# TiagoMSSantos/MobileRayTracer

Measured on AMD Instinct MI355X. Metric: Mrays/s + ms/frame, Conference OBJ 1920×1080 4spp, 1/2/4/8 GPU, higher is better.
Workload: dtype f32; 1 GPU; conference_1920x1080_4spp_pathtracer_depth5; rendered_pixels=2058240, spp=4, max_depth=5, samples_light=1, parallelism=single GPU

## Files before the change

### __graft_entry__.py

```python
import os
import subprocess
import sys

HERE = os.path.dirname(os.path.abspath(__file__))
if HERE not in sys.path:
    sys.path.insert(0, HERE)


def build() -> None:
    jobs = str(min(16, os.cpu_count() or 1))
    subprocess.run(["make", "-j", jobs, "-C", os.path.join(HERE, "mobileraytracer_amd", "csrc")], check=True)
    subprocess.run(["make", "-C", os.path.join(HERE, "oracle")], check=True)
    subprocess.run(["make", "-C", os.path.join(HERE, "tests", "cabi")], check=True)
    from mobileraytracer_amd import scenes
    scenes.conference()
    scenes.conference_flat()
    import mobileraytracer_amd
    from mobileraytracer_amd import _native
    _native.lib()


def smoke() -> None:
    import numpy as np
    import mobileraytracer_amd as m
    from oracle import oracle as O

    cfg = m.Config(width=64, height=64, shader=1, sceneIndex=0, device=0)
    with m.Renderer(cfg) as r:
        bm = np.zeros(64 * 64, np.int32)
        r.render_frame(bm)
        rays = r.get_total_casted_rays()
    ref, ref_rays = O.Oracle(64, 64, 1, 0).render(threads=4)
    assert np.array_equal(bm, ref), "Whitted Cornell bitmap differs from the oracle"
    assert rays == ref_rays, (rays, ref_rays)
    cfg = m.Config(width=64, height=64, shader=2, sceneIndex=0, samplesPixel=2, device=0)
    with m.Renderer(cfg) as r:
        bm = np.zeros(64 * 64, np.int32)
        r.render_frame(bm)
        prays = r.get_total_casted_rays()
        orig, dirs, keys, pixels = r.camera_rays()
        rgb = r.shade_rays(orig[:64], dirs[:64], keys[:64]).cpu().numpy()
        for q, px in enumerate(pixels[:64:2].cpu().numpy()):
            first = O.incremental_avg([float(x) for x in rgb[2 * q]], 0, 1)
            assert O.incremental_avg([float(x) for x in rgb[2 * q + 1]], first, 2) == bm[px], "shaded camera rays differ"
    ref, ref_prays = O.Oracle(64, 64, 2, 0, 2).render(threads=4)
    assert np.array_equal(bm, ref), "PathTracer Cornell bitmap differs from the oracle"
    assert prays == ref_prays, (prays, ref_prays)
    print("smoke ok: Cornell Whitted and PathTracer bit-exact, rays", rays, prays)


if __name__ == "__main__":
    build()
    smoke()
```

### include/mobilert_amd.h

```cpp
#ifndef MOBILERT_AMD_H
#define MOBILERT_AMD_H

#include <stddef.h>
#include <stdint.h>

#ifdef __cplusplus
extern "C" {
#endif

typedef struct mrt_renderer mrt_renderer;

typedef struct mrt_config {
    int32_t width;
    int32_t height;
    int32_t threads;
    int32_t shader;
    int32_t sceneIndex;
    int32_t samplesPixel;
    int32_t samplesLight;
    int32_t repeats;
    int32_t accelerator;
    int32_t printStdOut;
    const char *objFilePath;
    const char *mtlFilePath;
// ... 71 lines not shown
    int64_t worstCase;
    int64_t rayCap[MRT_QUEUE_LEVELS];
    int64_t shadowCap[MRT_QUEUE_LEVELS];
    int64_t requestedRays[MRT_QUEUE_LEVELS];
    int64_t requestedShadows[MRT_QUEUE_LEVELS];
} mrt_queue_info;

typedef struct mrt_queue_plan_request {
    int32_t levels;
    int32_t branching;
    int32_t samplesPixel;
    int32_t samplesLight;
    int32_t textured;
    int32_t segments;
    int32_t growthPct;
    int32_t slack;
    int32_t worstCase;
    int32_t hasDemand;
    int64_t pixelSlots;
    int64_t pathBudget;
    int64_t byteBudget;
    int32_t overflowMask;
    int32_t reserved;
    int64_t demandChunkSlots;
    int64_t demandPaths;
    int64_t segDemand[MRT_QUEUE_LEVELS];
    int64_t shadowSegDemand[MRT_QUEUE_LEVELS];
    int64_t prevChunkSlots;
    int64_t prevSegCap[MRT_QUEUE_LEVELS];
    int64_t prevShadowSegCap[MRT_QUEUE_LEVELS];
} mrt_queue_plan_request;

typedef struct mrt_queue_plan {
    int64_t chunkSlots;
    int64_t segCap[MRT_QUEUE_LEVELS];
    int64_t shadowSegCap[MRT_QUEUE_LEVELS];
    int64_t bytes;
    int64_t worstCase;
} mrt_queue_plan;

typedef struct mrt_blob {
    const char *name;
    const uint8_t *bytes;
    int64_t size;
} mrt_blob;

const char *mrt_last_error(void);
const char *mrt_build_stamp(void);
int mrt_create(const mrt_config *cfg, mrt_renderer **out);
int mrt_create_from_memory(const mrt_config *cfg, const char *obj, int64_t objLen, const char *mtl, int64_t mtlLen,
                           const char *cam, int64_t camLen, const mrt_blob *textures, int32_t nTextures,
                           mrt_renderer **out);
int64_t mrt_preview_arrays(const mrt_renderer *r, float *vertices, float *colors, float *camera);
void mrt_destroy(mrt_renderer *r);
int mrt_render_frame(mrt_renderer *r, int32_t *bitmap);
int mrt_render_frame_device(mrt_renderer *r, int32_t *d_bitmap, int32_t *d_packed, void *stream);
int mrt_unpack_gathered(mrt_renderer *r, const int32_t *d_gathered, int32_t *d_bitmap, void *stream);
int mrt_stop_render(mrt_renderer *r);
int32_t mrt_get_sample(const mrt_renderer *r);
uint64_t mrt_get_total_casted_rays(const mrt_renderer *r);
int mrt_get_scene_info(const mrt_renderer *r, mrt_scene_info *info);
int mrt_set_profiling(mrt_renderer *r, int32_t flags);
int mrt_get_frame_stats(const mrt_renderer *r, mrt_frame_stats *stats);
int mrt_get_queue_info(const mrt_renderer *r, mrt_queue_info *out, size_t size);
int64_t mrt_wave_log(mrt_renderer *r, uint64_t *out);
int mrt_set_camera(mrt_renderer *r, int32_t kind, const float *position, const float *lookAt, const float *up,
                   float a, float b);
int mrt_set_pixel_sampler(mrt_renderer *r, int32_t kind, float value);
int mrt_set_max_point(mrt_renderer *r, const float *maxPoint);
typedef struct mrt_view {
    int32_t kind;
    float position[3], lookAt[3], up[3];
    float a, b;
} mrt_view;
int mrt_render_views(mrt_renderer *r, const mrt_view *views, int32_t nViews, int32_t *bitmaps);
int mrt_render_views_device(mrt_renderer *r, const mrt_view *views, int32_t nViews,
                            int32_t *d_bitmaps, int32_t *d_packed, void *stream);
int mrt_set_tuning(mrt_renderer *r, int32_t key, int32_t value);
int mrt_get_tuning(const mrt_renderer *r, int32_t key, int32_t *value);
int mrt_primary_hits(mrt_renderer *r, int32_t *kind, int32_t *index, float *t);
int64_t mrt_triangle_bvh(const mrt_config *cfg, float *boxes, int32_t *offsets, int32_t *counts, int32_t *order);
int64_t mrt_walk_tree(const mrt_config *cfg, uint32_t *nodes, float *grid, int32_t *root);
int mrt_walk_stack(const mrt_config *cfg, int32_t *out);
int64_t mrt_plan_spill(int64_t threads, int32_t stackNeed, int64_t availBytes);
int64_t mrt_regular_grid(const mrt_config *cfg, int32_t kind, float *world, int32_t *start, int32_t *items);
int mrt_grid_box_test(int32_t kind, const float *prim, const float *box);
int64_t mrt_decode_texture(const char *path, int32_t *dims, uint8_t *texels);
int mrt_plan_queues(const mrt_queue_plan_request *request, mrt_queue_plan *plan);

int mrt_sample_tables(float *shader, float *sampler, float *trig);

int mrt_kat_slab(const float *boxes, const float *orig, const float *dir, int32_t n, int32_t *out);
int mrt_kat_triangle(const float *tris, const float *orig, const float *dir, int32_t n, int32_t *hit, float *t);
int mrt_kat_accumulate(const float *rgb, int32_t nSlots, int32_t spp, int32_t sampleBase, int32_t width,
                       int32_t height, int32_t mode, int32_t *bitmap, int32_t *launched);
int mrt_trace_rays(mrt_renderer *r, const float *orig, const float *dir, const float *dist, const int32_t *src,
                   int32_t n, int32_t any, int32_t *kind, int32_t *index, float *t);

typedef struct mrt_ray_batch {
    const float   *orig;
    const float   *dir;
    const float   *dist;
    const int32_t *src;
    int64_t origStride;
    int64_t dirStride;
    int64_t n;
} mrt_ray_batch;

int mrt_cast_rays_device(mrt_renderer *r, const mrt_ray_batch *rays, int32_t any,
                         int32_t *d_kind, int32_t *d_index, float *d_t, void *stream);

typedef struct mrt_hit_records {
    int32_t *kind; int32_t *index; float *t;
    float   *bary;
    float   *point;
    float   *normal;
    float   *texCoord;
    int32_t *material;
    float   *kd;
    float   *ks, *kt, *le;
    float   *ior;
} mrt_hit_records;

int mrt_cast_hits_device(mrt_renderer *r, const mrt_ray_batch *rays, const mrt_hit_records *out, size_t outSize,
                         void *stream);

int64_t mrt_scene_triangles(const mrt_config *cfg, float *geom, float *normals, float *texCoords, int32_t *material);
int64_t mrt_scene_planes(const mrt_config *cfg, float *normalPoint, int32_t *material);
int64_t mrt_scene_spheres(const mrt_config *cfg, float *centreSqRadius, int32_t *material);
int64_t mrt_scene_materials(const mrt_config *cfg, float *coeffs, int32_t *texture);
int64_t mrt_scene_lights(const mrt_config *cfg, int32_t *kind, float *geom, float *coeffs);


uint32_t mrt_path_key(uint32_t pixel, uint32_t sample);

typedef struct mrt_shade_batch {
    mrt_ray_batch rays;
    const uint32_t *key;
} mrt_shade_batch;

int mrt_shade_rays_device(mrt_renderer *r, const mrt_shade_batch *b, float *d_rgb, int64_t rgbStride,
                          uint64_t *raysOut, void *stream);

int64_t mrt_camera_rays_device(mrt_renderer *r, const mrt_view *view, int32_t sampleBase, int32_t spp,
                               float *d_orig, float *d_dir, uint32_t *d_key, int32_t *d_pixel, void *stream);

#ifdef __cplusplus
}
#endif

#endif
```

### mobileraytracer_amd/__init__.py

```python
import contextlib
import ctypes
import dataclasses
import threading
import time
from typing import List, Optional

import numpy as np

from . import _native

SHADER_WHITTED = 1
SHADER_PATH_TRACER = 2
ACC_BVH = 3
RAY_DEPTH_MAX = 6


@dataclasses.dataclass
class Config:
    width: int = 256
    height: int = 256
    threads: int = 1
    shader: int = SHADER_WHITTED
    sceneIndex: int = 0
    samplesPixel: int = 1
# ... 307 lines not shown
    def shade_rays(self, orig, dirs, keys=None, src=None):
        import torch

        device, n, orig, orig_stride, dirs, dir_stride = self._ray_tensors(orig, dirs)
        if keys is not None:
            if keys.device != device or keys.shape != (n,) or keys.dtype.is_floating_point:
                raise ValueError("keys: an integer tensor of shape (%d,) on %s" % (n, device))
            if keys.dtype == torch.uint32:
                keys = keys.contiguous().view(torch.int32)
            elif keys.dtype != torch.int32:
                keys = keys.to(torch.int64).to(torch.int32)
            keys = keys.contiguous()
        if src is not None:
            if src.device != device or src.shape != (n, 2):
                raise ValueError("src: a tensor of shape (%d, 2) on %s" % (n, device))
            src = src.to(torch.int32).contiguous()
        rgb = torch.empty((n, 3), dtype=torch.float32, device=device)
        if n == 0:
            return rgb
        with self._query_stream_of(device) as stream:
            self.shade_rays_device(orig.data_ptr(), dirs.data_ptr(), n, d_key=keys.data_ptr() if keys is not None else 0,
                                   d_src=src.data_ptr() if src is not None else 0, orig_stride=orig_stride,
                                   dir_stride=dir_stride, d_rgb=rgb.data_ptr(), stream=stream)
        return rgb

    def camera_rays(self, camera=None, sample_base: int = 0, spp: Optional[int] = None):
        import torch

        spp = int(spp) if spp else max(1, self.config.samplesPixel)
        n = self.scene_info()["pixelSlots"] * spp
        device = torch.device("cuda", self.config.device if self.config.device >= 0 and not self.config.devices
                              else torch.cuda.current_device())
        orig = torch.empty((n, 3), dtype=torch.float32, device=device)
        dirs = torch.empty((n, 3), dtype=torch.float32, device=device)
        keys = torch.empty(n, dtype=torch.int32, device=device).view(torch.uint32)
        pixels = torch.empty(n, dtype=torch.int32, device=device)
        if n == 0:
            return orig, dirs, keys, pixels
        view = self._views([camera]) if camera is not None else None
        got = self._lib.mrt_camera_rays_device(self._h, view, int(sample_base), spp, orig.data_ptr(), dirs.data_ptr(),
                                               keys.data_ptr(), pixels.data_ptr(),
                                               ctypes.c_void_p(torch.cuda.current_stream(device).cuda_stream or None))
        if got != n:
            _native.check(-1 if got < 0 else 0)
            raise RuntimeError("mrt_camera_rays_device returned %d paths, %d expected" % (got, n))
        return orig, dirs, keys, pixels

    def close(self) -> None:
        if getattr(self, "_h", None):
            self._lib.mrt_destroy(self._h)
            self._h = None

    def __del__(self):
        self.close()

    def __enter__(self):
        return self

    def __exit__(self, *exc):
        self.close()


def walk_tree(config: Config):
    lib = _native.lib()
    c = config.to_c()
    n = lib.mrt_walk_tree(ctypes.byref(c), None, None, None)
    if n < 0:
        raise RuntimeError(lib.mrt_last_error().decode())
    grid = np.empty(6, np.float32)
    root = np.empty(3, np.int32)
    lib.mrt_walk_tree(ctypes.byref(c), None, _ptr(grid), _ptr(root))
    nodes = np.empty((n, 4 * int(root[2])), np.uint32)
    if lib.mrt_walk_tree(ctypes.byref(c), _ptr(nodes), _ptr(grid), _ptr(root)) != n:
        raise RuntimeError(lib.mrt_last_error().decode())
    return nodes, grid, root


def walk_stack(config: Config) -> dict:
    out = np.zeros(6, np.int32)
    c = config.to_c()
    _native.check(_native.lib().mrt_walk_stack(ctypes.byref(c), _ptr(out)))
    return {"need": int(out[0]), "quantized": bool(out[1]), "refDepth": int(out[2]), "walkDepth": int(out[3]),
            "wideDepth": int(out[4]), "spillDepth": int(out[5])}


def plan_spill(threads: int, stack_need: int, avail_bytes: int = 0) -> int:
    n = _native.lib().mrt_plan_spill(int(threads), int(stack_need), int(avail_bytes))
    if n < 0:
        raise RuntimeError(_native.lib().mrt_last_error().decode())
    return int(n)


def triangle_bvh(config: Config):
    lib = _native.lib()
    c = config.to_c()
    n = lib.mrt_triangle_bvh(ctypes.byref(c), None, None, None, None)
    if n < 0:
        raise RuntimeError(lib.mrt_last_error().decode())
    boxes = np.empty((n, 6), np.float32)
    off, cnt = np.empty(n, np.int32), np.empty(n, np.int32)
    order = np.full((n + 1) // 2, -1, np.int32)
    n2 = lib.mrt_triangle_bvh(ctypes.byref(c), _ptr(boxes), _ptr(off), _ptr(cnt), _ptr(order))
    if n2 != n:
        raise RuntimeError(lib.mrt_last_error().decode())
    return boxes, off, cnt, order[:int(cnt[0])] if n == 1 else order


def _scene_arrays(name, config, shapes):
    lib = _native.lib()
    fn = getattr(lib, name)
    c = config.to_c()
    n = fn(ctypes.byref(c), *([None] * len(shapes)))
    if n < 0:
        raise RuntimeError(lib.mrt_last_error().decode())
    arrays = [np.zeros((n,) + shape, dtype) for dtype, shape in shapes]
    if fn(ctypes.byref(c), *[_ptr(a) for a in arrays]) != n:
        raise RuntimeError(lib.mrt_last_error().decode())
    return arrays


def scene_triangles(config: Config):
    return tuple(_scene_arrays("mrt_scene_triangles", config, [(np.float32, (3, 3)), (np.float32, (3, 3)),
                                                               (np.float32, (3, 2)), (np.int32, ())]))


def scene_planes(config: Config):
    return tuple(_scene_arrays("mrt_scene_planes", config, [(np.float32, (2, 3)), (np.int32, ())]))


def scene_spheres(config: Config):
    return tuple(_scene_arrays("mrt_scene_spheres", config, [(np.float32, (4,)), (np.int32, ())]))


def scene_materials(config: Config):
    return tuple(_scene_arrays("mrt_scene_materials", config, [(np.float32, (13,)), (np.int32, ())]))


def scene_lights(config: Config):
    return tuple(_scene_arrays("mrt_scene_lights", config, [(np.int32, ()), (np.float32, (3, 3)), (np.float32, (13,))]))


def plan_queues(levels: int, branching: int, pixel_slots: int, samples_pixel: int = 1, samples_light: int = 1,
                textured: bool = False, path_budget: int = 0, byte_budget: int = 0, growth_pct: int = 0,
                slack: int = -1, worst_case: bool = False, demand: Optional[dict] = None,
                previous: Optional[dict] = None) -> dict:
    q = _native.MrtQueuePlanRequest()
    q.levels, q.branching, q.samplesPixel, q.samplesLight = levels, branching, samples_pixel, samples_light
    q.textured, q.segments, q.growthPct, q.slack = int(textured), 0, growth_pct, slack
    q.worstCase, q.pixelSlots, q.pathBudget, q.byteBudget = int(worst_case), pixel_slots, path_budget, byte_budget
    if demand is not None:
        q.hasDemand = 1
        q.overflowMask = int(demand["mask"])
        q.demandChunkSlots = int(demand["chunkSlots"])
        q.demandPaths = int(demand["paths"])
        for i, v in enumerate(demand["seg"]):
            q.segDemand[i] = int(v)
        for i, v in enumerate(demand["shadowSeg"]):
            q.shadowSegDemand[i] = int(v)
    if previous is not None:
        q.prevChunkSlots = int(previous["chunkSlots"])
        for i, v in enumerate(previous["segCap"]):
            q.prevSegCap[i] = int(v)
        for i, v in enumerate(previous["shadowSegCap"]):
            q.prevShadowSegCap[i] = int(v)
    plan = _native.MrtQueuePlan()
    _native.check(_native.lib().mrt_plan_queues(ctypes.byref(q), ctypes.byref(plan)))
# ... 121 lines not shown
```

### mobileraytracer_amd/_native.py

```python
import ctypes
import os

_HERE = os.path.dirname(os.path.abspath(__file__))
LIB_PATH = os.environ.get("MOBILERT_LIB") or os.path.join(_HERE, "libmobilert_amd.so")

EXPORTED_SYMBOLS = (
    "mrt_last_error", "mrt_build_stamp", "mrt_create", "mrt_destroy", "mrt_render_frame", "mrt_render_frame_device",
    "mrt_unpack_gathered", "mrt_stop_render", "mrt_get_sample", "mrt_get_total_casted_rays",
    "mrt_get_scene_info", "mrt_set_profiling", "mrt_get_frame_stats", "mrt_primary_hits", "mrt_set_tuning",
    "mrt_get_tuning", "mrt_triangle_bvh", "mrt_walk_tree", "mrt_decode_texture", "mrt_kat_slab", "mrt_kat_triangle",
    "mrt_trace_rays", "mrt_sample_tables", "mrt_regular_grid", "mrt_grid_box_test", "mrt_create_from_memory",
    "mrt_preview_arrays", "mrt_wave_log", "mrt_set_camera", "mrt_set_pixel_sampler", "mrt_set_max_point",
    "mrt_android_read_file", "mrt_android_initialize", "mrt_android_render_into_bitmap",
    "mrt_android_render_into_bitmap_cb", "mrt_android_wait_render", "mrt_android_start_render",
    "mrt_android_stop_render", "mrt_android_finish_render", "mrt_android_state", "mrt_android_fps",
    "mrt_android_time_renderer", "mrt_android_sample", "mrt_android_number_of_lights", "mrt_android_resize",
    "mrt_android_vertices", "mrt_android_colors", "mrt_android_camera", "mrt_android_reset",
    "mrt_get_queue_info", "mrt_plan_queues", "mrt_render_views", "mrt_render_views_device",
    "mrt_kat_accumulate", "mrt_cast_rays_device", "mrt_walk_stack", "mrt_plan_spill",
    "mrt_path_key", "mrt_shade_rays_device", "mrt_camera_rays_device",
    "mrt_cast_hits_device", "mrt_scene_triangles", "mrt_scene_planes", "mrt_scene_spheres", "mrt_scene_materials",
    "mrt_scene_lights",
    "RayTrace", "stopRender",
)


class MrtConfig(ctypes.Structure):
    _fields_ = [
        ("width", ctypes.c_int32), ("height", ctypes.c_int32), ("threads", ctypes.c_int32),
        ("shader", ctypes.c_int32), ("sceneIndex", ctypes.c_int32), ("samplesPixel", ctypes.c_int32),
        ("samplesLight", ctypes.c_int32), ("repeats", ctypes.c_int32), ("accelerator", ctypes.c_int32),
        ("printStdOut", ctypes.c_int32),
        ("objFilePath", ctypes.c_char_p), ("mtlFilePath", ctypes.c_char_p), ("camFilePath", ctypes.c_char_p),
        ("maxDepth", ctypes.c_int32), ("rankIndex", ctypes.c_int32), ("rankCount", ctypes.c_int32),
        ("device", ctypes.c_int32), ("cull", ctypes.c_int32), ("maxPathsPerPass", ctypes.c_int32),
        ("progressive", ctypes.c_int32), ("devices", ctypes.POINTER(ctypes.c_int32)), ("deviceCount", ctypes.c_int32),
    ]


class MrtAndroidConfig(ctypes.Structure):
    _fields_ = [(n, ctypes.c_int32) for n in (
        "scene", "shader", "accelerator", "width", "height", "samplesPixel", "samplesLight")] + [
        ("objFilePath", ctypes.c_char_p)]


class MrtBlob(ctypes.Structure):
    _fields_ = [("name", ctypes.c_char_p), ("bytes", ctypes.c_char_p), ("size", ctypes.c_int64)]


class MrtView(ctypes.Structure):
    _fields_ = [("kind", ctypes.c_int32), ("position", ctypes.c_float * 3), ("lookAt", ctypes.c_float * 3),
                ("up", ctypes.c_float * 3), ("a", ctypes.c_float), ("b", ctypes.c_float)]


class MrtRayBatch(ctypes.Structure):
    _fields_ = [("orig", ctypes.c_void_p), ("dir", ctypes.c_void_p), ("dist", ctypes.c_void_p), ("src", ctypes.c_void_p),
                ("origStride", ctypes.c_int64), ("dirStride", ctypes.c_int64), ("n", ctypes.c_int64)]


HIT_FIELDS = (("kind", "int32", 1), ("index", "int32", 1), ("t", "float32", 1), ("bary", "float32", 2),
              ("point", "float32", 3), ("normal", "float32", 3), ("texCoord", "float32", 2), ("material", "int32", 1),
              ("kd", "float32", 3), ("ks", "float32", 3), ("kt", "float32", 3), ("le", "float32", 3), ("ior", "float32", 1))


class MrtHitRecords(ctypes.Structure):
    _fields_ = [(name, ctypes.c_void_p) for name, _, _ in HIT_FIELDS]


class MrtShadeBatch(ctypes.Structure):
    _fields_ = [("rays", MrtRayBatch), ("key", ctypes.c_void_p)]


class MrtSceneInfo(ctypes.Structure):
    _fields_ = [(n, ctypes.c_int64) for n in (
        "triangles", "lights", "planes", "spheres", "materials", "triangleNodes", "triangleBvhDepth",
        "pixelSlots", "pixelSlotsMax", "deviceBytes", "shadowStreamConcurrent", "shadowStreamsTried", "deviceCount")]


class MrtFrameStats(ctypes.Structure):
    _fields_ = [
        ("rays", ctypes.c_uint64), ("shadowRays", ctypes.c_uint64), ("primaryRays", ctypes.c_uint64),
        ("nodeRecords", ctypes.c_uint64), ("triTests", ctypes.c_uint64),
        ("shadowNodeRecords", ctypes.c_uint64), ("shadowTriTests", ctypes.c_uint64),
        ("traceMs", ctypes.c_double), ("shadowMs", ctypes.c_double), ("frameMs", ctypes.c_double),
        ("traceLaunches", ctypes.c_int64), ("shadowLaunches", ctypes.c_int64),
        ("shadeMs", ctypes.c_double),
        ("levelRays", ctypes.c_uint64 * 16), ("levelShadowRays", ctypes.c_uint64 * 16),
        ("levelTraceMs", ctypes.c_double * 16), ("levelShadowMs", ctypes.c_double * 16),
        ("maxNodeRecordsPerRay", ctypes.c_uint64),
        ("walkedRays", ctypes.c_uint64), ("shadedVertices", ctypes.c_uint64), ("shadeLaunches", ctypes.c_int64),
        ("leafRecords", ctypes.c_uint64), ("shadowLeafRecords", ctypes.c_uint64),
        ("levelNodeRecords", ctypes.c_uint64 * 16), ("levelTriTests", ctypes.c_uint64 * 16),
        ("levelLeafRecords", ctypes.c_uint64 * 16),
        ("fusedMs", ctypes.c_double), ("fusedLaunches", ctypes.c_int64),
        ("levelShadedVertices", ctypes.c_uint64 * 16),
        ("shadowOccluded", ctypes.c_uint64),
        ("walkPhases", ctypes.c_uint64 * 16),
        ("packetWaveRecords", ctypes.c_uint64 * 3),
    ]


QUEUE_LEVELS = 16


class MrtQueueInfo(ctypes.Structure):
    _fields_ = [(n, ctypes.c_int64) for n in (
        "chunkSlots", "passes", "queueBytes", "budgetBytes", "replans", "replansLastFrame", "worstCase")] + [
        (n, ctypes.c_int64 * QUEUE_LEVELS) for n in ("rayCap", "shadowCap", "requestedRays", "requestedShadows")]


class MrtQueuePlanRequest(ctypes.Structure):
    _fields_ = [(n, ctypes.c_int32) for n in (
        "levels", "branching", "samplesPixel", "samplesLight", "textured", "segments", "growthPct", "slack",
        "worstCase", "hasDemand")] + [
        ("pixelSlots", ctypes.c_int64), ("pathBudget", ctypes.c_int64), ("byteBudget", ctypes.c_int64),
        ("overflowMask", ctypes.c_int32), ("reserved", ctypes.c_int32),
        ("demandChunkSlots", ctypes.c_int64), ("demandPaths", ctypes.c_int64),
        ("segDemand", ctypes.c_int64 * QUEUE_LEVELS), ("shadowSegDemand", ctypes.c_int64 * QUEUE_LEVELS),
        ("prevChunkSlots", ctypes.c_int64),
        ("prevSegCap", ctypes.c_int64 * QUEUE_LEVELS), ("prevShadowSegCap", ctypes.c_int64 * QUEUE_LEVELS)]


class MrtQueuePlan(ctypes.Structure):
    _fields_ = [("chunkSlots", ctypes.c_int64), ("segCap", ctypes.c_int64 * QUEUE_LEVELS),
                ("shadowSegCap", ctypes.c_int64 * QUEUE_LEVELS), ("bytes", ctypes.c_int64),
                ("worstCase", ctypes.c_int64)]


def _preload_torch_hip_runtime():
    import importlib.util
    spec = importlib.util.find_spec("torch")
    if spec is None or not spec.origin:
        return
    rt = os.path.join(os.path.dirname(spec.origin), "lib", "libamdhip64.so")
    if os.path.exists(rt):
        ctypes.CDLL(rt, mode=ctypes.RTLD_GLOBAL)


def load_library(path=LIB_PATH):
    if not os.path.exists(path):
        raise ImportError(
            f"{path} is missing: build it with `python -c 'import __graft_entry__ as g; g.build()'` "
            "(the MI355X path has no CPU fallback)")
    _preload_torch_hip_runtime()
    lib = ctypes.CDLL(path)
    P = ctypes.POINTER
    vp = ctypes.c_void_p
    sig = {
        "mrt_last_error": (ctypes.c_char_p, []),
        "mrt_build_stamp": (ctypes.c_char_p, []),
        "mrt_create": (ctypes.c_int, [P(MrtConfig), P(vp)]),
        "mrt_destroy": (None, [vp]),
        "mrt_render_frame": (ctypes.c_int, [vp, vp]),
        "mrt_render_frame_device": (ctypes.c_int, [vp, vp, vp, vp]),
        "mrt_render_views": (ctypes.c_int, [vp, P(MrtView), ctypes.c_int32, vp]),
        "mrt_render_views_device": (ctypes.c_int, [vp, P(MrtView), ctypes.c_int32, vp, vp, vp]),
        "mrt_unpack_gathered": (ctypes.c_int, [vp, vp, vp, vp]),
        "mrt_stop_render": (ctypes.c_int, [vp]),
        "mrt_get_sample": (ctypes.c_int32, [vp]),
        "mrt_get_total_casted_rays": (ctypes.c_uint64, [vp]),
        "mrt_get_scene_info": (ctypes.c_int, [vp, P(MrtSceneInfo)]),
        "mrt_set_profiling": (ctypes.c_int, [vp, ctypes.c_int32]),
        "mrt_get_frame_stats": (ctypes.c_int, [vp, P(MrtFrameStats)]),
        "mrt_get_queue_info": (ctypes.c_int, [vp, vp, ctypes.c_size_t]),
        "mrt_plan_queues": (ctypes.c_int, [P(MrtQueuePlanRequest), P(MrtQueuePlan)]),
        "mrt_wave_log": (ctypes.c_int64, [vp, vp]),
        "mrt_primary_hits": (ctypes.c_int, [vp, vp, vp, vp]),
        "mrt_set_tuning": (ctypes.c_int, [vp, ctypes.c_int32, ctypes.c_int32]),
        "mrt_get_tuning": (ctypes.c_int, [vp, ctypes.c_int32, ctypes.POINTER(ctypes.c_int32)]),
        "mrt_triangle_bvh": (ctypes.c_int64, [vp, vp, vp, vp, vp]),
        "mrt_walk_tree": (ctypes.c_int64, [vp, vp, vp, vp]),
        "mrt_walk_stack": (ctypes.c_int, [vp, vp]),
        "mrt_plan_spill": (ctypes.c_int64, [ctypes.c_int64, ctypes.c_int32, ctypes.c_int64]),
        "mrt_decode_texture": (ctypes.c_int64, [ctypes.c_char_p, vp, vp]),
        "mrt_regular_grid": (ctypes.c_int64, [vp, ctypes.c_int32, vp, vp, vp]),
        "mrt_grid_box_test": (ctypes.c_int, [ctypes.c_int32, vp, vp]),
        "mrt_create_from_memory": (ctypes.c_int, [P(MrtConfig), ctypes.c_char_p, ctypes.c_int64, ctypes.c_char_p,
                                                  ctypes.c_int64, ctypes.c_char_p, ctypes.c_int64, vp, ctypes.c_int32,
                                                  P(vp)]),
        "mrt_preview_arrays": (ctypes.c_int64, [vp, vp, vp, vp]),
        "mrt_set_camera": (ctypes.c_int, [vp, ctypes.c_int32, vp, vp, vp, ctypes.c_float, ctypes.c_float]),
        "mrt_set_pixel_sampler": (ctypes.c_int, [vp, ctypes.c_int32, ctypes.c_float]),
        "mrt_set_max_point": (ctypes.c_int, [vp, vp]),
        "mrt_android_read_file": (None, [ctypes.c_char_p, ctypes.c_char_p, ctypes.c_int64]),
        "mrt_android_initialize": (ctypes.c_int32, [P(MrtAndroidConfig)]),
        "mrt_android_render_into_bitmap": (None, [vp, ctypes.c_int32]),
        "mrt_android_render_into_bitmap_cb": (None, [vp, ctypes.c_int32, vp, vp]),
        "mrt_android_wait_render": (None, []),
        "mrt_android_start_render": (None, [ctypes.c_int32]),
        "mrt_android_stop_render": (None, [ctypes.c_int32]),
        "mrt_android_finish_render": (None, []),
        "mrt_android_state": (ctypes.c_int32, []),
        "mrt_android_fps": (ctypes.c_float, []),
        "mrt_android_time_renderer": (ctypes.c_int64, []),
        "mrt_android_sample": (ctypes.c_int32, []),
        "mrt_android_number_of_lights": (ctypes.c_int32, []),
        "mrt_android_resize": (ctypes.c_int32, [ctypes.c_int32]),
        "mrt_android_vertices": (ctypes.c_int64, [vp]),
        "mrt_android_colors": (ctypes.c_int64, [vp]),
        "mrt_android_camera": (ctypes.c_int64, [vp]),
        "mrt_android_reset": (None, []),
        "mrt_sample_tables": (ctypes.c_int, [vp, vp, vp]),
        "mrt_kat_slab": (ctypes.c_int, [vp, vp, vp, ctypes.c_int32, vp]),
        "mrt_kat_triangle": (ctypes.c_int, [vp, vp, vp, ctypes.c_int32, vp, vp]),
        "mrt_kat_accumulate": (ctypes.c_int, [vp] + [ctypes.c_int32] * 6 + [vp, P(ctypes.c_int32)]),
        "mrt_trace_rays": (ctypes.c_int, [vp, vp, vp, vp, vp, ctypes.c_int32, ctypes.c_int32, vp, vp, vp]),
        "mrt_cast_rays_device": (ctypes.c_int, [vp, P(MrtRayBatch), ctypes.c_int32, vp, vp, vp, vp]),
        "mrt_cast_hits_device": (ctypes.c_int, [vp, P(MrtRayBatch), P(MrtHitRecords), ctypes.c_size_t, vp]),
        "mrt_scene_triangles": (ctypes.c_int64, [vp, vp, vp, vp, vp]),
        "mrt_scene_planes": (ctypes.c_int64, [vp, vp, vp]),
        "mrt_scene_spheres": (ctypes.c_int64, [vp, vp, vp]),
        "mrt_scene_materials": (ctypes.c_int64, [vp, vp, vp]),
        "mrt_scene_lights": (ctypes.c_int64, [vp, vp, vp, vp]),
        "mrt_path_key": (ctypes.c_uint32, [ctypes.c_uint32, ctypes.c_uint32]),
        "mrt_shade_rays_device": (ctypes.c_int, [vp, P(MrtShadeBatch), vp, ctypes.c_int64, P(ctypes.c_uint64), vp]),
        "mrt_camera_rays_device": (ctypes.c_int64, [vp, P(MrtView), ctypes.c_int32, ctypes.c_int32, vp, vp, vp, vp, vp]),
    }
    for name, (res, args) in sig.items():
        if os.environ.get("MOBILERT_LIB") and not hasattr(lib, name):
            continue
        fn = getattr(lib, name)
        fn.restype = res
        fn.argtypes = args
    return lib


_LIB = None


def lib():
    global _LIB
    if _LIB is None:
        _LIB = load_library()
    return _LIB


def source_stamp():
    import hashlib
    d = os.path.join(_HERE, "csrc")
    srcs = ["mrt_scene.cpp", "mrt_grid.cpp", "mrt_texture.cpp", "mrt_android.cpp", "mrt_queue_plan.cpp", "mrt_kernels.hip",
            "mrt_renderer.hip",
            "mrt_common.hpp", "mrt_device.hpp", "mrt_kernels.hpp", "mrt_trace_ww.hpp", "mrt_trace_packet.hpp",
            "mrt_scene.hpp", "mrt_queue_plan.hpp", "../../include/mobilert_amd.h", "../../include/mobilert_amd.hpp",
            "../../include/mobilert_android.h"]
    h = hashlib.sha256()
    for f in srcs:
        with open(os.path.join(d, f), "rb") as fh:
            h.update(fh.read())
    return h.hexdigest()[:16]


def build_is_current(library=None):
    return (library or lib()).mrt_build_stamp().decode() == source_stamp()


# ... 4 lines not shown
```

### mobileraytracer_amd/csrc/mrt_kernels.hip

```cpp
#include "mrt_kernels.hpp"
#include "mrt_trace_ww.hpp"
#include "mrt_trace_packet.hpp"

#include <algorithm>
#include <atomic>
#include <utility>

namespace mrt {

__device__ __forceinline__ int laneId() { return static_cast<int>(threadIdx.x & 63u); }

__device__ __forceinline__ int waveExclusiveScan(int v, int* total) {
    const int lane = laneId();
    int x = v;
#pragma unroll
    for (int off = 1; off < 64; off <<= 1) {
        const int y = __shfl_up(x, off, 64);
        if (lane >= off) x += y;
    }
    *total = __shfl(x, 63, 64);
    return x - v;
}

__device__ __forceinline__ int waveAlloc(int* counter, int n) {
// ... 51 lines not shown
__device__ __forceinline__ void cameraRayOf(const GCamera& c, float u, float v, float devU, float devV, uint32_t key,
                                            float4* o4, float4* d4) {
    v3 origin, dir;
    if (c.kind == 1) {
        const float rf = (u - 0.5F) * c.hFov;
        const v3 right = c.right * rf + c.right * devU;
        const float uf = (0.5F - v) * c.vFov;
        const v3 up = c.up * uf + c.up * devV;
        origin = (c.position + right) + up;
        dir = c.direction;
    } else {
        const float rf = fastArcTan(c.hFov * (u - 0.5F)) + devU;
        const v3 right = c.right * rf;
        const float uf = fastArcTan(c.vFov * (0.5F - v)) + devV;
        const v3 up = c.up * uf;
        const v3 dest = ((c.position + c.direction) + right) + up;
        origin = c.position;
        dir = normalize(dest - c.position);
    }
    *o4 = make_float4(origin.x, origin.y, origin.z, bitsf(key));
    *d4 = make_float4(dir.x, dir.y, dir.z, bitsf(kNoPrim));
}
static_assert(sizeof(GCamera) == 64, "cameraRay reads a view's camera as 16 dwords");
template <bool kViews = false>
__device__ __forceinline__ void cameraRay(const RaygenArgs& a, int p, float4* o4, float4* d4) {
    int slot = a.slotBase + p / a.spp;
    int view = 0;
    if constexpr (kViews) {
        view = slot / a.viewSlots;
        slot -= view * a.viewSlots;
    }
    const int s = p % a.spp;
    int x, y;
    slotToXY(a.map, slot, &x, &y);
    const uint32_t pixelIndex = static_cast<uint32_t>(y * a.width + x);
    const uint32_t key = pathKey(pixelIndex, static_cast<uint32_t>(a.sampleBase + s));
    const float invW = 1.0F / static_cast<float>(a.width);
    const float invH = 1.0F / static_cast<float>(a.height);
    const float pixW = 0.5F / static_cast<float>(a.width);
    const float pixH = 0.5F / static_cast<float>(a.height);
    const float u = static_cast<float>(x) * invW;
    const float v = static_cast<float>(y) * invH;
    float r1 = a.constJitter, r2 = a.constJitter;
    if (a.tableJitter != 0) {
        const float2 j = a.jitter[sampleBlock(key, 0u)];
        r1 = j.x;
        r2 = j.y;
    }
    const float devU = (r1 - 0.5F) * 2.0F * pixW;
    const float devV = (r2 - 0.5F) * 2.0F * pixH;
    if constexpr (kViews) {
        const int first = __builtin_amdgcn_readfirstlane(view);
        if (__ballot(view != first) == 0) {
            ConstU32* const w = (ConstU32*)(a.cams) + 16 * first;
            const float4 c0 = sload4f(w), c1 = sload4f(w + 4), c2 = sload4f(w + 8), c3 = sload4f(w + 12);
            pinSgprs(c0);
            pinSgprs(c1);
            pinSgprs(c2);
            pinSgprs(c3);
            const GCamera c{v3{c0.x, c0.y, c0.z}, v3{c0.w, c1.x, c1.y}, v3{c1.z, c1.w, c2.x}, v3{c2.y, c2.z, c2.w},
                            c3.x, c3.y, __float_as_int(c3.z), 0};
            cameraRayOf(c, u, v, devU, devV, key, o4, d4);
        } else {
            const GCamera c = a.cams[view];
            cameraRayOf(c, u, v, devU, devV, key, o4, d4);
        }
    } else {
        cameraRayOf(a.cam, u, v, devU, devV, key, o4, d4);
    }
}

template <bool kViews>
__global__ __launch_bounds__(256) void k_raygen(RaygenArgs a, Level lv, int* counters) {
    const int p = static_cast<int>(blockIdx.x * blockDim.x + threadIdx.x);
    if (p == 0) denseCounts(counters, 1, false, a.nPaths, lv.segCap);
    if (p >= a.nPaths) return;
    float4 o4, d4;
    cameraRay<kViews>(a, p, &o4, &d4);
    lv.rO[p] = o4;
    lv.rD[p] = d4;
    lv.tree[p] = 1u;
}

constexpr int kWalkThreads = 256;

template <bool kCount>
__device__ __forceinline__ void reduceCounts(const TravCount& cnt, unsigned long long* stats, int nodesStat,
                                             int trisStat, int leavesStat) {
    unsigned long long n = cnt.nodes, t = cnt.tris, l = cnt.leaves;
    for (int off = 32; off > 0; off >>= 1) {
        n += __shfl_down(n, off, 64);
        t += __shfl_down(t, off, 64);
        l += __shfl_down(l, off, 64);
    }
    if (laneId() == 0) {
        atomicAdd(stats + nodesStat, n);
        atomicAdd(stats + trisStat, t);
        atomicAdd(stats + leavesStat, l);
    }
}

__device__ __forceinline__ void reducePhases(const TravCount& cnt, unsigned long long* stats, int kind) {
    const uint32_t v[6] = {cnt.innerIters, cnt.innerLanes, cnt.leafIters, cnt.leafLanes, cnt.triIters, cnt.triLanes};
#pragma unroll
    for (int k = 0; k < 6; ++k) {
        unsigned long long x = v[k];
        for (int off = 32; off > 0; off >>= 1) x += __shfl_down(x, off, 64);
        if (laneId() == 0 && x != 0) atomicAdd(stats + kStatPhases + 6 * kind + k, x);
    }
    const uint32_t w[2] = {cnt.innerIdle, cnt.innerDone};
#pragma unroll
    for (int k = 0; k < 2; ++k) {
        unsigned long long x = w[k];
        for (int off = 32; off > 0; off >>= 1) x += __shfl_down(x, off, 64);
        if (laneId() == 0 && x != 0) atomicAdd(stats + kStatPhases + 12 + 2 * kind + k, x);
    }
}

__device__ __forceinline__ void waveLog(const TravCount& cnt, unsigned long long* stats, int kind, int level,
                                        unsigned long long t0) {
    unsigned long long n = cnt.nodes, r = cnt.rays;
    for (int off = 32; off > 0; off >>= 1) {
        n += __shfl_down(n, off, 64);
        r += __shfl_down(r, off, 64);
    }
    const int wave = static_cast<int>(blockIdx.x * (kWalkThreads / 64) + threadIdx.x / 64);
    if (laneId() == 0 && wave < kWaveLogWaves && level < kMaxLevels) {
        unsigned long long* e = stats + kNumStats + ((static_cast<size_t>(kind) * kMaxLevels + level) * kWaveLogWaves + wave) * 4;
        e[0] = t0;
        e[1] = __builtin_amdgcn_s_memrealtime();
        e[2] = r;
        e[3] = n;
    }
}

template <int kCull>
__device__ __forceinline__ auto makeWalkStack(int2* ldsStack, int2* gstack, int gdepth) {
    if constexpr (kCull == kCullFast || kCull == kCullCertified)
        return makeKeyStack<kWalkThreads>(ldsStack, gstack, gdepth);
    else
        return makeRefStack<kWalkThreads>(ldsStack, gstack, gdepth);
}

#ifndef MRT_WALK_WAVES
#define MRT_WALK_WAVES 6
#endif
#ifndef MRT_SHADOW_WAVES
#define MRT_SHADOW_WAVES MRT_WALK_WAVES
#endif
template <bool kCount, int kVariant, int kCull>
__global__ __launch_bounds__(kWalkThreads, MRT_WALK_WAVES) void k_trace(DScene s, Level lv, int* counters, int level,
                                                            int2* gstack, int gdepth, unsigned long long* stats) {
    __shared__ int2 ldsStack[kWalkStack * kWalkThreads];
    auto st = makeWalkStack<kCull>(ldsStack, gstack, gdepth);
    const unsigned long long t0 = kCount ? __builtin_amdgcn_s_memrealtime() : 0ull;
    const SegMap map = segMap(counters, level, false, lv.segCap);
    int* fetch = counters + kCntFetchShards + level * kMaxFetchShards * kFetchStride;
    TravCount cnt{0u, 0u};
    if (kVariant == 1) {
        __shared__ QNode4 ldsTop[kWalkTop];
        __shared__ int tailBest[kWalkThreads];
        stageTop<kWalkThreads>(s, ldsTop);
        traceWhileWhile<false, kCount, kCull>(s, lv.rO, lv.rD, lv.hit, map, fetch, st, &cnt, ldsTop, tailBest);
    }
    while (kVariant == 0) {
        int base = 0;
        if (laneId() == 0) base = atomicAdd(fetch, 64);
        base = __shfl(base, 0, 64);
        if (base >= map.total()) break;
        const int v = base + laneId();
        if (v < map.total()) {
            const int i = map.phys(v);
            const float4 o4 = lv.rO[i];
            const float4 d4 = lv.rD[i];
            const Best b = closestHit(s, xyz(o4), xyz(d4), fbits(d4.w), st, &cnt);
            lv.hit[i] = make_float4(b.t, b.u, b.v, bitsf(b.code));
        }
    }
    if (kCount) {
        reduceCounts<kCount>(cnt, stats, kStatNodes, kStatTris, kStatLeaves);
        reduceCounts<kCount>(cnt, stats, kStatLevelNodes + level - 1, kStatLevelTris + level - 1, kStatLevelLeaves + level - 1);
        reducePhases(cnt, stats, 0);
        atomicMax(stats + kStatMaxNodesRay, static_cast<unsigned long long>(cnt.rayMax));
        waveLog(cnt, stats, 0, level, t0);
    }
}

template <bool kViews>
struct PacketRaysStore {
    const RaygenArgs* a;
    Level lv;
    __device__ __forceinline__ void operator()(int i, float4* o4, float4* d4) const {
        cameraRay<kViews>(*a, i, o4, d4);
        if (a->storeRays != 0) {
            lv.rO[i] = *o4;
            lv.rD[i] = *d4;
            lv.tree[i] = 1u;
        }
    }
};

template <bool kCount, int kCull, int kGen>
__global__ __launch_bounds__(kWalkThreads, kGen ? 7 : 8) void k_trace_packet(DScene s, Level lv, int* counters, int level,
                                                                   int2* gstack, int gdepth, unsigned long long* stats,
                                                                   RaygenArgs ra) {
    __shared__ int2 ldsStack[kWalkStack * kWalkThreads];
    __shared__ int waveStacks[kWalkThreads / 64][kPacketStack];
    auto st = makeWalkStack<kCull>(ldsStack, gstack, gdepth);
    const unsigned long long t0 = kCount ? __builtin_amdgcn_s_memrealtime() : 0ull;
// ... 1481 lines not shown
```

### mobileraytracer_amd/csrc/mrt_kernels.hpp

```cpp
#pragma once

#include "mrt_device.hpp"

namespace mrt {

constexpr int kShaderWhitted = 1;
constexpr int kShaderPathTracer = 2;
constexpr int kShaderDepthMap = 3;
constexpr int kShaderDiffuse = 4;
constexpr int kShaderNoShadows = 5;
constexpr int kMaxLevels = 16;
constexpr int kTraceVariants = 2;
constexpr int kDefaultTraceVariant = 1;
constexpr int kAccNaive = 1;
constexpr int kAccGrid = 2;
constexpr int kAccBVH = 3;
constexpr int kTopNodesMax = 64 * 4 / kWalkWidth;

#ifndef MRT_QUEUE_SEGS
#define MRT_QUEUE_SEGS 8
#endif
constexpr int kQueueSegs = MRT_QUEUE_SEGS;
constexpr int kCntSegStride = 64;
constexpr int kCntPairs = 0;
constexpr int kCntOverflow = kQueueSegs * kCntSegStride;
constexpr int kPacketStack = 128;
#ifndef MRT_WALK_CURSORS
#define MRT_WALK_CURSORS 8
#endif
constexpr int kMaxFetchShards = MRT_WALK_CURSORS;
constexpr int kFetchStride = 32;
constexpr int kCntFetchShards = kCntOverflow + kFetchStride;
constexpr int kNumCounters = kCntFetchShards + 2 * kMaxLevels * kMaxFetchShards * kFetchStride;
MRT_HD constexpr int cntRays(int level, int seg = 0) { return kCntPairs + seg * kCntSegStride + 2 * (level - 1); }
MRT_HD constexpr int cntShadows(int level, int seg = 0) { return kCntPairs + seg * kCntSegStride + 2 * level + 1; }
static_assert(kQueueSegs >= 1 && kQueueSegs <= kMaxFetchShards, "queue segments: one work cursor each at most");
static_assert(cntShadows(kMaxLevels) < kCntSegStride, "a segment's pairs within its line");

constexpr int kStatRays = 0;
constexpr int kStatShadowRays = 1;
constexpr int kStatPrimary = 2;
constexpr int kStatNodes = 3;
constexpr int kStatTris = 4;
constexpr int kStatOverflow = 5;
constexpr int kStatNodesShadow = 6;
constexpr int kStatTrisShadow = 7;
constexpr int kStatLevelRays = 8;
constexpr int kStatLevelShadows = 8 + kMaxLevels;
constexpr int kStatMaxNodesRay = 8 + 2 * kMaxLevels;
constexpr int kStatSkipped = kStatMaxNodesRay + 1;
constexpr int kStatShaded = kStatSkipped + 1;
constexpr int kStatShadeLaunches = kStatShaded + 1;
constexpr int kStatLeaves = kStatShadeLaunches + 1;
constexpr int kStatLeavesShadow = kStatLeaves + 1;
constexpr int kStatLevelNodes = kStatLeavesShadow + 1;
constexpr int kStatLevelTris = kStatLevelNodes + kMaxLevels;
constexpr int kStatLevelLeaves = kStatLevelTris + kMaxLevels;
constexpr int kStatLevelShaded = kStatLevelLeaves + kMaxLevels;
constexpr int kStatOccluded = kStatLevelShaded + kMaxLevels;
constexpr int kStatPhases = kStatOccluded + 1;
constexpr int kStatPacket = kStatPhases + 16;
constexpr int kStatReqSegRays = kStatPacket + 3;
constexpr int kStatReqSegShadows = kStatReqSegRays + kMaxLevels;
constexpr int kStatReqRays = kStatReqSegShadows + kMaxLevels;
constexpr int kStatReqShadows = kStatReqRays + kMaxLevels;
constexpr int kNumStats = kStatReqShadows + kMaxLevels;
constexpr int kWaveLogWaves = 8192;
constexpr int kWaveLogEntries = 2 * kMaxLevels * kWaveLogWaves * 4;

struct Level {
    float4* rO;
    float4* rD;
    uint32_t* tree;
    float4* hit;
    int4* vtx;
    float4* res;
    float4* sO;
    float4* sD;
    float4* sC;
    float4* kd;
    float4* last;
    int cap;
    int shadowCap;
    int segCap;
    int shadowSegCap;
};

struct TexLevel {
    const int4* vtx;
    const float4* kd;
    const float4* last;
    int cap;
    int pad;
};

struct PixelMap {
    const int4* rect;
    const int* prefix;
    int nUnits;
    int pad;
// ... 164 lines not shown
```

### mobileraytracer_amd/csrc/mrt_renderer.hip

```cpp
#include <algorithm>
#include <atomic>
#include <chrono>
#include <cmath>
#include <condition_variable>
#include <functional>
#include <cstdio>
#include <cstdlib>
#include <cstring>
#include <deque>
#include <exception>
#include <future>
#include <memory>
#include <mutex>
#include <stdexcept>
#include <map>
#include <sstream>
#include <string>
#include <thread>
#include <unordered_map>
#include <vector>

#include "mobilert_amd.h"
#include "mobilert_amd.hpp"
#include "mrt_kernels.hpp"
#include "mrt_queue_plan.hpp"
#include "mrt_scene.hpp"

namespace {

#define MRT_HIP(x)                                                                              \
    do {                                                                                        \
        const hipError_t e_ = (x);                                                              \
        if (e_ != hipSuccess) throw std::runtime_error(std::string(#x) + ": " + hipGetErrorString(e_)); \
    } while (0)

thread_local std::string gLastError;

struct DeviceMem {
    std::vector<void*> ptrs;
    size_t total = 0;
    template <class T>
    T* alloc(size_t n) {
        if (n == 0) n = 1;
        void* p = nullptr;
        MRT_HIP(hipMalloc(&p, n * sizeof(T)));
        ptrs.push_back(p);
        total += n * sizeof(T);
        return static_cast<T*>(p);
    }
    template <class T>
    T* upload(const std::vector<T>& v, hipStream_t st) {
        T* p = alloc<T>(v.size());
        if (!v.empty()) MRT_HIP(hipMemcpyAsync(p, v.data(), v.size() * sizeof(T), hipMemcpyHostToDevice, st));
        return p;
    }
    void release() {
        for (void* p : ptrs) (void)hipFree(p);
        ptrs.clear();
        total = 0;
    }
    ~DeviceMem() { release(); }
};

#ifndef MRT_RAY_ROT_SWEEPS
#define MRT_RAY_ROT_SWEEPS 1
#endif
constexpr int kRayRotSweeps = MRT_RAY_ROT_SWEEPS;
constexpr size_t kFrameTreeCache = 4;
struct FrameTree {
    std::vector<mrt::HBVHNode> nodes;
    std::vector<double> cost;
};
struct Fnv64 {
    uint64_t h = 1469598103934665603ull;
    void add(const void* p, size_t n) {
        const auto* b = static_cast<const unsigned char*>(p);
        for (size_t i = 0; i < n; ++i) h = (h ^ b[i]) * 1099511628211ull;
    }
    template <class T>
    void pod(const T& v) { add(&v, sizeof(v)); }
};
std::vector<mrt::HBVHNode> frameWalkTree(const std::vector<mrt::HBVHNode>& wn, const mrt::HScene& sc, const mrt::GCamera& cam,
                                         int width, int height, int maxDepth, std::vector<double>* cost) {
    cost->clear();
    const char* ce = std::getenv("MOBILERT_COLLAPSE");
    if (ce != nullptr && (std::string(ce) == "area" || std::string(ce) == "greedy")) return wn;
    if (wn.empty() || sc.triangles.empty() || width <= 0 || height <= 0) {
        cost->assign(wn.size(), 0.0);
        return wn;
    }
    const char* re = std::getenv("MOBILERT_RAY_ROT");
    const int sweeps = re != nullptr ? std::atoi(re) : kRayRotSweeps;
    Fnv64 f;
    f.add(wn.data(), wn.size() * sizeof(mrt::HBVHNode));
    for (const mrt::HTriangle& t : sc.triangles) {
        f.pod(t.AC);
        f.pod(t.AB);
        f.pod(t.A);
        f.pod(t.mat);
    }
    for (const mrt::HMaterial& m : sc.materials) {
        f.pod(m.Le);
        f.pod(m.Kd);
        f.pod(m.Ks);
    }
    for (const mrt::HLight& l : sc.lights) {
        f.pod(l.kind);
        f.pod(l.tri.A);
        f.pod(l.tri.AB);
        f.pod(l.tri.AC);
    }
    f.pod(cam);
    const int dims[4] = {width, height, maxDepth, sweeps};
    f.pod(dims);
    using Entry = std::shared_ptr<const FrameTree>;
    static std::mutex mu;
    static std::unordered_map<uint64_t, std::shared_future<Entry>> cache;
    static std::deque<uint64_t> order;
    std::promise<Entry> mine;
    std::shared_future<Entry> pending;
    {
        std::lock_guard<std::mutex> lock(mu);
        const auto it = cache.find(f.h);
        if (it != cache.end()) {
            pending = it->second;
        } else {
            cache.emplace(f.h, mine.get_future().share());
            order.push_back(f.h);
            while (order.size() > kFrameTreeCache) {
                cache.erase(order.front());
                order.pop_front();
            }
        }
    }
    if (pending.valid()) {
        const Entry e = pending.get();
        *cost = e->cost;
        return e->nodes;
    }
    try {
        auto e = std::make_shared<FrameTree>();
        const std::vector<mrt::SampleRay> rays = mrt::sampleFrameRays(wn, sc, cam, maxDepth);
        e->nodes = sweeps > 0 ? mrt::rotateForRays(wn, rays, sweeps) : wn;
        e->cost = mrt::sampleRayNodeCosts(e->nodes, rays);
        mine.set_value(e);
        *cost = e->cost;
        return e->nodes;
    } catch (...) {
        mine.set_exception(std::current_exception());
        std::lock_guard<std::mutex> lock(mu);
        cache.erase(f.h);
        order.erase(std::remove(order.begin(), order.end(), f.h), order.end());
        throw;
    }
}

int bvhDepth(const std::vector<mrt::HBVHNode>& nodes) {
    if (nodes.empty()) return 0;
    int best = 0;
    std::vector<std::pair<int, int>> st{{0, 1}};
    while (!st.empty()) {
        const auto [i, d] = st.back();
        st.pop_back();
        best = std::max(best, d);
        const mrt::HBVHNode& n = nodes[static_cast<size_t>(i)];
        if (n.numPrimitives == 0 && nodes.size() > 1) {
            st.push_back({n.indexOffset, d + 1});
            st.push_back({n.indexOffset + 1, d + 1});
        }
    }
    return best;
}

int wideDepth(bool quantized, const mrt::GRoot& root, const std::vector<mrt::QNode4>& qn) {
    int depth4 = 0;
    std::vector<std::pair<int32_t, int>> w;
    if (quantized && root.count > 0 && root.ref >= 0) w.push_back({root.ref, 1});
    while (!w.empty()) {
        const auto [i, dep] = w.back();
        w.pop_back();
        depth4 = std::max(depth4, dep);
        for (int32_t c : qn[static_cast<size_t>(i)].ref)
            if (c >= 0 && c != mrt::kEmptyChild) w.push_back({c, dep + 1});
    }
    return depth4;
}

int walkStackNeed(int binaryDepth, int depth4) {
    return std::max(binaryDepth + 2, (mrt::kWalkWidth - 1) * depth4 + 2);
}

int spillDepth(int stackNeed) { return std::max(1, stackNeed - mrt::kLdsStackMin); }

float4 f4(mrt::v3 v, float w) { return make_float4(v.x, v.y, v.z, w); }
float asFloat(int32_t i) {
    float f;
    std::memcpy(&f, &i, 4);
    return f;
}

}

std::vector<int32_t> mrt::parseDeviceList(const char* s) {
    std::vector<int32_t> out;
    if (s == nullptr) return out;
    std::string item;
    std::istringstream in(s);
    while (std::getline(in, item, ',')) {
        char* end = nullptr;
        const long v = std::strtol(item.c_str(), &end, 10);
        if (item.empty() || end != item.c_str() + item.size() || v < 0 || v > 0x7fffffffL)
            throw std::runtime_error(std::string("MOBILERT_DEVICES: bad ordinal '") + item + "'");
        out.push_back(static_cast<int32_t>(v));
    }
    return out;
}

namespace {

class ShardPool {
public:
    explicit ShardPool(const std::vector<int>& devices) : n_(static_cast<int>(devices.size())), err_(devices.size()) {
        for (int i = 1; i < n_; ++i) th_.emplace_back([this, i, d = devices[static_cast<size_t>(i)]] { loop(i, d); });
    }
    ~ShardPool() {
        {
            std::lock_guard<std::mutex> lock(mu_);
            quit_ = true;
        }
        wake_.notify_all();
        for (std::thread& t : th_) t.join();
    }
    ShardPool(const ShardPool&) = delete;
    ShardPool& operator=(const ShardPool&) = delete;

    void run(const std::function<void(int)>& job) {
        std::lock_guard<std::mutex> serial(runMu_);
// ... 36 lines not shown
                if (bound != hipSuccess)
                    throw std::runtime_error(std::string("shard worker: hipSetDevice: ") + hipGetErrorString(bound));
                (*job)(i);
            } catch (...) {
                err_[static_cast<size_t>(i)] = std::current_exception();
            }
            {
                std::lock_guard<std::mutex> lock(mu_);
                if (--pending_ == 0) done_.notify_one();
            }
        }
    }

    const int n_;
    std::mutex runMu_, mu_;
    std::condition_variable wake_, done_;
    std::vector<std::thread> th_;
    std::vector<std::exception_ptr> err_;
    const std::function<void(int)>* job_ = nullptr;
    uint64_t gen_ = 0;
    int pending_ = 0;
    bool quit_ = false;
};

}

struct mrt_renderer {
    mrt_config cfg{};
    std::string objPath, mtlPath, camPath;
    int maxDepth = mrt::kRayDepthMaxDefault;
    int shader = mrt::kShaderWhitted;
    int nLevels = 1;
    mrt::v3 maxPoint{1.0F, 1.0F, 1.0F};
    int pixelSampler = -1;
    float pixelConst = 0.5F;
    int rankIndex = 0, rankCount = 1;
    int device = 0;
    int shadowConcurrent = 0;
    int shadowTries = 0;
    std::vector<hipStream_t> spareStreams;
    unsigned long long* spinTimes = nullptr;
    hipEvent_t joinIn = nullptr, joinOut = nullptr;

    mrt::GCamera cam{};
    mrt::DScene ds{};
    std::vector<int32_t> triOrder, planeOrder, sphereOrder;
    int64_t nTri = 0, nLights = 0, nPlanes = 0, nSpheres = 0, nMats = 0, nTriNodes = 0;
    int triDepth = 0, maxBvhDepth = 0;
    int stackNeed = 0;

    std::vector<std::vector<int4>> unitsByRank;
    std::vector<std::vector<int>> prefixByRank;
    std::vector<mrt::PixelMap> mapByRank;
    int nSlots = 0, maxSlots = 0;

    DeviceMem sceneMem, queueMem, frameMem;
    struct Pipe {
        mrt::Level levels[mrt::kMaxLevels]{};
        mrt::TexLevel* texLevels = nullptr;
        int* counters = nullptr;
        unsigned long long* stats = nullptr;
        int2* gstack = nullptr;
        int2* gstackShadow = nullptr;
        hipStream_t shadowStream = nullptr;
        std::vector<hipEvent_t> syncPool;
        std::vector<hipEvent_t> evPool;
        size_t evCount = 0;
    } pipe;
    int chunkSlots = 0;
    mrt_queue_plan plan{};
    int64_t planBudget = 0;
    int queueBudgetMiB = 0;
    int queueGrowthPct = mrt::kPlanGrowthPct;
    int queueSlack = mrt::kPlanSlack;
    int deviceShare = 1;
    bool planStale = false;
    int64_t replans = 0, replansFrame = 0;
    int64_t reqSegRays[mrt::kMaxLevels] = {}, reqSegShadows[mrt::kMaxLevels] = {};
    int64_t reqRays[mrt::kMaxLevels] = {}, reqShadows[mrt::kMaxLevels] = {};
    int overflowMask = 0;
    int64_t reqPaths = 0;
    int gdepth = 0;
    int traceThreads = 0, workGrid = 0;
    int cus = 0;
    int shadeGridPerCU = -1;
    int32_t* dBitmap = nullptr;
    int32_t* dBackup = nullptr;
    size_t backupN = 0;
    int views = 1;
    const mrt::GCamera* batchCams = nullptr;
    mrt::GCamera* dViewCams = nullptr;
    size_t viewCamsN = 0;
    std::vector<mrt::GCamera> hostViewCams;
    int32_t* dViewBitmaps = nullptr;
    size_t viewBitmapsN = 0;
    DeviceMem queryMem;
    mrt::QueryTables queryTables{};
    bool queryReady = false;
    int64_t planSlots = 0;
    int planSpp = 0;
    struct ShadeBatch {
        mrt::QueryRays rays;
        const uint32_t* keys;
        float* rgb;
        long long rgbStride;
        int64_t n;
    };
    const ShadeBatch* shade = nullptr;
    hipStream_t stream = nullptr;
    int overlap = 1;
    int skipLast = 1;
    int shadowGridPct = 0;
    int fuseL1Mode = -1;
    int genL1 = 2;
    int resolveAcc = 1;
    int shadeWaitsShadow = 0;
    int refill = 0;
    int64_t shadeLaunches = 0;
    bool walkSkipped = false;
    bool fusedL1 = false;
    int lastShadowRender = 1;
    int walkGridCap = 0;
    unsigned long long* hostStats = nullptr;
    bool countersClean = false, statsClean = false;

    bool keepHost = false;
    std::vector<mrt::HTriangle> hostTris;
    std::vector<mrt::HMaterial> hostMats;

    std::atomic<bool> stopFlag{false};
    std::atomic<int32_t> sample{0};
    std::atomic<uint64_t> totalRays{0};
    int profileFlags = 0;
    mrt_frame_stats last{};

    std::vector<std::unique_ptr<mrt_renderer>> peers;
    int32_t* dOwnPacked = nullptr;
    int32_t* dGathered = nullptr;
    std::unique_ptr<ShardPool> shardPool;

    ~mrt_renderer() {
        if (hostStats != nullptr) (void)hipHostFree(hostStats);
        for (hipEvent_t e : pipe.evPool) (void)hipEventDestroy(e);
        for (hipEvent_t e : pipe.syncPool) (void)hipEventDestroy(e);
        if (pipe.shadowStream != nullptr) (void)hipStreamDestroy(pipe.shadowStream);
        for (hipStream_t s : spareStreams) (void)hipStreamDestroy(s);
        if (joinIn != nullptr) (void)hipEventDestroy(joinIn);
        if (joinOut != nullptr) (void)hipEventDestroy(joinOut);
        if (stream != nullptr) (void)hipStreamDestroy(stream);
    }
};

namespace {

void frameUnits(int W, int H, int rankCount, std::vector<std::vector<int4>>* units,
                std::vector<std::vector<int>>* prefix) {
    const int tilesPerSide = static_cast<int>(std::sqrt(static_cast<double>(mrt::kNumberOfTiles)));
    const int bx = W / tilesPerSide, by = H / tilesPerSide;
    if (bx <= 0 || by <= 0) throw std::runtime_error("width and height must be >= 16 (Renderer.cpp:33-38)");
    const int domainSize = (W / bx) * (H / by);
    const int resolution = W * H;
    std::vector<int> blocks;
    for (int j = 0; j < mrt::kNumberOfTiles; ++j) {
        const float tile = static_cast<float>(j) / static_cast<float>(mrt::kNumberOfTiles);
        const int rb = static_cast<int>(::roundf(tile * static_cast<float>(domainSize)));
        if (std::find(blocks.begin(), blocks.end(), rb) == blocks.end()) blocks.push_back(rb);
    }
    std::vector<int4> all;
    std::vector<int> owner;
    for (size_t t = 0; t < blocks.size(); ++t) {
        const int rb = blocks[t];
        const int pixel = rb * bx % resolution;
        const int startY = ((pixel / W) * by) % H;
        const int startX = pixel % W;
        for (int b = 0; b * 8 < by; ++b) {
            int h = std::min(8, by - 8 * b);
            const int y0 = startY + 8 * b;
            while (h > 0 && (y0 + h - 1) * W + startX + bx - 1 >= resolution) --h;
            if (h > 0) {
                all.push_back(make_int4(startX, y0, bx, h));
                owner.push_back(static_cast<int>((t + static_cast<size_t>(b)) % static_cast<size_t>(rankCount)));
            }
        }
    }
    units->assign(static_cast<size_t>(rankCount), {});
    prefix->assign(static_cast<size_t>(rankCount), {});
    for (size_t u = 0; u < all.size(); ++u) (*units)[static_cast<size_t>(owner[u])].push_back(all[u]);
    for (int k = 0; k < rankCount; ++k) {
        int acc = 0;
        for (const int4& u : (*units)[static_cast<size_t>(k)]) {
            (*prefix)[static_cast<size_t>(k)].push_back(acc);
            acc += u.z * u.w;
        }
    }
}

int unitSlots(const std::vector<int4>& units) {
    int acc = 0;
    for (const int4& u : units) acc += u.z * u.w;
    return acc;
}

void buildUnits(mrt_renderer* r) {
    frameUnits(r->cfg.width, r->cfg.height, r->rankCount, &r->unitsByRank, &r->prefixByRank);
    r->maxSlots = 0;
    for (int k = 0; k < r->rankCount; ++k) {
        const int acc = unitSlots(r->unitsByRank[static_cast<size_t>(k)]);
        if (k == r->rankIndex) r->nSlots = acc;
        r->maxSlots = std::max(r->maxSlots, acc);
    }
    r->mapByRank.clear();
    for (int k = 0; k < r->rankCount; ++k) {
        mrt::PixelMap m{};
        m.rect = r->sceneMem.upload(r->unitsByRank[static_cast<size_t>(k)], r->stream);
        m.prefix = r->sceneMem.upload(r->prefixByRank[static_cast<size_t>(k)], r->stream);
        m.nUnits = static_cast<int>(r->unitsByRank[static_cast<size_t>(k)].size());
        r->mapByRank.push_back(m);
    }
}

void slotToXYHost(const std::vector<int4>& units, const std::vector<int>& prefix, int slot, int* x, int* y) {
    const auto it = std::upper_bound(prefix.begin(), prefix.end(), slot);
    const size_t u = static_cast<size_t>(it - prefix.begin()) - 1;
    const int off = slot - prefix[u];
    *x = units[u].x + off / units[u].w;
    *y = units[u].y + off % units[u].w;
}

void uploadScene(mrt_renderer* r, mrt::HScene& sc) {
    using namespace mrt;
    hipStream_t st = r->stream;
    std::vector<HBVHNode> pn = buildBVH(&sc.planes, &r->planeOrder);
    std::vector<HBVHNode> sn = buildBVH(&sc.spheres, &r->sphereOrder);
    std::vector<HBVHNode> tn = buildBVH(&sc.triangles, &r->triOrder);
    std::vector<double> rayCost;
    const std::vector<HBVHNode> wn =
        frameWalkTree(walkTreeOver(tn), sc, r->cam, r->cfg.width, r->cfg.height, r->maxDepth, &rayCost);
    r->nTri = static_cast<int64_t>(sc.triangles.size());
    r->nPlanes = static_cast<int64_t>(sc.planes.size());
    r->nSpheres = static_cast<int64_t>(sc.spheres.size());
    r->nLights = static_cast<int64_t>(sc.lights.size());
    r->nMats = static_cast<int64_t>(sc.materials.size());
    r->nTriNodes = static_cast<int64_t>(tn.size());
    r->triDepth = std::max(bvhDepth(tn), bvhDepth(wn));
    r->maxBvhDepth = std::max({r->triDepth, bvhDepth(pn), bvhDepth(sn)});

    if (r->keepHost) {
        r->hostTris = sc.triangles;
        r->hostMats = sc.materials;
    }
    std::vector<GNode> g;
    DScene& d = r->ds;
    const std::vector<uint32_t> conesRef = triangleConeWords(tn, sc.triangles);
    std::vector<QNode4> qn;
    d.qEnabled = toQuantizedBVH4(wn, sc.triangles.size(), &d.triRoot, kTopNodesMax, &d.triTop, &d.qgrid, &qn, nullptr,
                                 rayCost.empty() ? nullptr : &rayCost) ? 1 : 0;
    if (d.qEnabled == 0 || qn.empty()) qn.resize(1);
    d.triQNodes = r->sceneMem.upload(qn, st);
    {
        static_assert(kWalkWidth == 4, "packet nodes: 4 children");
        std::vector<float> qf(32 * qn.size(), 0.0F);
        for (size_t k = 0; k < qn.size(); ++k) {
            const QNode4& q = qn[k];
            for (int c = 0; c < kWalkWidth; ++c) {
                const uint32_t w0 = q.q[3 * c], w1 = q.q[3 * c + 1], w2 = q.q[3 * c + 2];
                const uint32_t v[6] = {w0 & 0xFFFFu, w1 & 0xFFFFu, w2 & 0xFFFFu, w0 >> 16, w1 >> 16, w2 >> 16};
                for (int j = 0; j < 6; ++j) qf[32 * k + 6 * static_cast<size_t>(c) + static_cast<size_t>(j)] = static_cast<float>(v[j]);
                std::memcpy(&qf[32 * k + 24 + static_cast<size_t>(c)], &q.ref[c], sizeof(int32_t));
            }
        }
        d.triQNodesF = r->sceneMem.upload(qf, st);
    }
    r->stackNeed = walkStackNeed(r->maxBvhDepth, wideDepth(d.qEnabled != 0, d.triRoot, qn));
    {
        std::string err;
        if (planSpillBytes(r->traceThreads, spillDepth(r->stackNeed), 0, &err) < 0) throw std::runtime_error(err);
    }
    toDeviceBVH(tn, sc.triangles.size(), &g, &d.triRootRef, 0, nullptr, &conesRef);
    {
        std::vector<float4> lb(std::max<size_t>(1, 3 * sc.triangles.size()), make_float4(0.0F, 0.0F, 0.0F, 0.0F));
        for (const HBVHNode& n : tn) {
            if (n.numPrimitives <= 0) continue;
            const size_t f = static_cast<size_t>(n.indexOffset);
            float c[6];
            leafCullRecord(sc.triangles, f, f + static_cast<size_t>(n.numPrimitives), n.box, c);
            lb[3 * f] = make_float4(n.box.mn.x, n.box.mn.y, n.box.mn.z, n.box.mx.x);
            lb[3 * f + 1] = make_float4(n.box.mx.y, n.box.mx.z, c[0], c[1]);
            lb[3 * f + 2] = make_float4(c[2], c[3], c[4], c[5]);
        }
        d.leafBoxes = r->sceneMem.upload(lb, st);
    }
    d.triNodes = r->sceneMem.upload(g, st);
    toDeviceBVH(pn, sc.planes.size(), &g, &d.planeRoot);
    d.planeNodes = r->sceneMem.upload(g, st);
    toDeviceBVH(sn, sc.spheres.size(), &g, &d.sphereRoot);
    d.sphereNodes = r->sceneMem.upload(g, st);

    std::vector<float4> v;
    v.reserve(sc.triangles.size() * 3);
    for (const HTriangle& t : sc.triangles) {
        v.push_back(f4(t.A, 0.0F));
        v.push_back(f4(t.AB, 0.0F));
        v.push_back(f4(t.AC, 0.0F));
    }
    d.triGeom = r->sceneMem.upload(v, st);
    v.clear();
    for (const HTriangle& t : sc.triangles) {
        v.push_back(f4(t.nA, asFloat(t.mat)));
        v.push_back(f4(t.nB, 0.0F));
        v.push_back(f4(t.nC, 0.0F));
    }
    d.triShade = r->sceneMem.upload(v, st);
    v.clear();
    for (const HTriangle& t : sc.triangles) {
        const bool flat = std::memcmp(&t.nA, &t.nB, sizeof(t.nA)) == 0 && std::memcmp(&t.nA, &t.nC, sizeof(t.nA)) == 0;
        v.push_back(f4(t.nA, asFloat(static_cast<int32_t>((static_cast<uint32_t>(t.mat + 1) << 1) | (flat ? 1u : 0u)))));
    }
    d.triHead = r->sceneMem.upload(v, st);
    v.clear();
    d.textured = 0;
    for (const HMaterial& m : sc.materials) d.textured += (m.texId >= 0 && !sc.textures.empty()) ? 1 : 0;
    if (d.textured != 0) {
        for (const HTriangle& t : sc.triangles) {
            v.push_back(make_float4(t.tA.x, t.tA.y, t.tB.x, t.tB.y));
            v.push_back(make_float4(t.tC.x, t.tC.y, 0.0F, 0.0F));
        }
        d.triTex = r->sceneMem.upload(v, st);
        v.clear();
        std::vector<int4> info;
        std::vector<uint8_t> bytes;
        for (const HTexture& t : sc.textures) {
            info.push_back(make_int4(t.width, t.height, t.channels, static_cast<int>(bytes.size())));
            bytes.insert(bytes.end(), t.texels.begin(), t.texels.end());
        }
        d.texInfo = r->sceneMem.upload(info, st);
        d.texels = r->sceneMem.upload(bytes, st);
    } else {
        d.triTex = nullptr;
        d.texInfo = nullptr;
        d.texels = nullptr;
// ... 1443 lines not shown
        r->ds.cull = value;
        return 0;
    }
    if (key == 3 && (value == 0 || value == 1)) {
        r->overlap = value;
        return 0;
    }
    if (key == 7 && (value == 0 || value == 1)) {
        r->skipLast = value;
        return 0;
    }
    if (key == 5 && (value == 0 || value == 1)) {
        r->ds.anyOrder = value;
        return 0;
    }
    if (key == 11 && value >= -1 && value <= 64) {
        r->shadeGridPerCU = value;
        return 0;
    }
    if (key == 10 && (value == 0 || value == 1)) {
        r->ds.leanShade = value;
        return 0;
    }
    if (key == 9 && value >= 0 && value <= 64) {
        r->refill = value;
        return 0;
    }
    if (key == 8 && (value == 0 || value == 1)) {
        r->ds.tailDonate = value;
        return 0;
    }
    if (key == 16 && (value == 0 || value == 1)) {
        if (value == 1 && r->stackNeed > mrt::kPacketStack) {
            gLastError = "packet walk: the walk tree needs a deeper stack";
            return -1;
        }
        r->ds.packet = value;
        return 0;
    }
    if (key == 17 && value >= -1 && value <= 1) {
        r->fuseL1Mode = value;
        return 0;
    }
    if (key == 27 && (value == 0 || value == 1)) {
        r->lastShadowRender = value;
        return 0;
    }
    if (key == 33 && value >= 0 && value <= 2) {
        r->genL1 = value;
        return 0;
    }
    if (key == 34 && (value == 0 || value == 1)) {
        r->resolveAcc = value;
        return 0;
    }
    if (key == 35 && (value == 0 || value == 1)) {
        r->shadeWaitsShadow = value;
        return 0;
    }

    if (key == 28 && value >= 0 && value <= 65536) {
        r->walkGridCap = value;
        return 0;
    }
    if (key == 6 && value >= 0 && value <= 100) {
        r->shadowGridPct = value;
        return 0;
    }
    if (key == 37 && value >= 0 && value <= (1 << 20)) {
        r->queueBudgetMiB = value;
        r->planStale = true;
        return 0;
    }
    if (key == 38 && value >= 1 && value <= 100000) {
        r->queueGrowthPct = value;
        r->planStale = true;
        return 0;
    }
    if (key == 39 && value >= 0 && value <= (1 << 24)) {
        r->queueSlack = value;
        r->planStale = true;
        return 0;
    }
    gLastError = "unknown tuning key/value";
    return -1;
}

int64_t mrt_triangle_bvh(const mrt_config* cfg, float* boxes, int32_t* offsets, int32_t* counts, int32_t* order) {
    using namespace mrt;
    int64_t n = -1;
    const int rc = guarded([&] {
        HScene sc;
        if (cfg->sceneIndex >= 0 && cfg->sceneIndex <= 3) {
            sc = builtinScene(cfg->sceneIndex);
        } else {
            std::string err;
            if (!loadObjScene(cfg->objFilePath ? cfg->objFilePath : "", cfg->mtlFilePath ? cfg->mtlFilePath : "", &sc,
                              &err))
                throw std::runtime_error(err);
        }
        std::vector<int32_t> perm;
        const std::vector<HBVHNode> nodes = buildBVH(&sc.triangles, &perm);
        n = static_cast<int64_t>(nodes.size());
        if (boxes == nullptr) return;
        for (size_t i = 0; i < nodes.size(); ++i) {
            const HBVHNode& b = nodes[i];
            const float v[6] = {b.box.mn.x, b.box.mn.y, b.box.mn.z, b.box.mx.x, b.box.mx.y, b.box.mx.z};
            std::memcpy(boxes + 6 * i, v, sizeof(v));
            offsets[i] = b.indexOffset;
            counts[i] = b.numPrimitives;
        }
        std::memcpy(order, perm.data(), perm.size() * sizeof(int32_t));
    });
    return rc == 0 ? n : -1;
}

int64_t mrt_scene_triangles(const mrt_config* cfg, float* geom, float* normals, float* texCoords, int32_t* material) {
    int64_t n = -1;
    const int rc = guarded([&] {
        const mrt::HScene sc = sceneOf(cfg);
        for (size_t i = 0; i < sc.triangles.size(); ++i) {
            const mrt::HTriangle& t = sc.triangles[i];
            if (geom != nullptr) {
                put3(geom + 9 * i, t.A);
                put3(geom + 9 * i + 3, t.AB);
                put3(geom + 9 * i + 6, t.AC);
            }
            if (normals != nullptr) {
                put3(normals + 9 * i, t.nA);
                put3(normals + 9 * i + 3, t.nB);
                put3(normals + 9 * i + 6, t.nC);
            }
            if (texCoords != nullptr) {
                const float tc[6] = {t.tA.x, t.tA.y, t.tB.x, t.tB.y, t.tC.x, t.tC.y};
                std::memcpy(texCoords + 6 * i, tc, sizeof(tc));
            }
            if (material != nullptr) material[i] = t.mat;
        }
        n = static_cast<int64_t>(sc.triangles.size());
    });
    return rc == 0 ? n : -1;
}

int64_t mrt_scene_planes(const mrt_config* cfg, float* normalPoint, int32_t* material) {
    int64_t n = -1;
    const int rc = guarded([&] {
        const mrt::HScene sc = sceneOf(cfg);
        for (size_t i = 0; i < sc.planes.size(); ++i) {
            if (normalPoint != nullptr) {
                put3(normalPoint + 6 * i, sc.planes[i].normal);
                put3(normalPoint + 6 * i + 3, sc.planes[i].point);
            }
            if (material != nullptr) material[i] = sc.planes[i].mat;
        }
        n = static_cast<int64_t>(sc.planes.size());
    });
    return rc == 0 ? n : -1;
}

int64_t mrt_scene_spheres(const mrt_config* cfg, float* centreSqRadius, int32_t* material) {
    int64_t n = -1;
    const int rc = guarded([&] {
        const mrt::HScene sc = sceneOf(cfg);
        for (size_t i = 0; i < sc.spheres.size(); ++i) {
            if (centreSqRadius != nullptr) {
                put3(centreSqRadius + 4 * i, sc.spheres[i].center);
                centreSqRadius[4 * i + 3] = sc.spheres[i].sqRadius;
            }
            if (material != nullptr) material[i] = sc.spheres[i].mat;
        }
        n = static_cast<int64_t>(sc.spheres.size());
    });
    return rc == 0 ? n : -1;
}

int64_t mrt_scene_materials(const mrt_config* cfg, float* coeffs, int32_t* texture) {
    int64_t n = -1;
    const int rc = guarded([&] {
        const mrt::HScene sc = sceneOf(cfg);
        for (size_t i = 0; i < sc.materials.size(); ++i) {
            if (coeffs != nullptr) putMaterial(coeffs + 13 * i, sc.materials[i]);
            if (texture != nullptr) texture[i] = sc.materials[i].texId;
        }
        n = static_cast<int64_t>(sc.materials.size());
    });
    return rc == 0 ? n : -1;
}

int64_t mrt_scene_lights(const mrt_config* cfg, int32_t* kind, float* geom, float* coeffs) {
    int64_t n = -1;
    const int rc = guarded([&] {
        const mrt::HScene sc = sceneOf(cfg);
        for (size_t i = 0; i < sc.lights.size(); ++i) {
            const mrt::HLight& l = sc.lights[i];
            const bool area = l.kind == mrt::kAreaLight;
            if (kind != nullptr) kind[i] = l.kind;
            if (geom != nullptr) {
                put3(geom + 9 * i, area ? l.tri.A : l.position);
                put3(geom + 9 * i + 3, area ? l.tri.AB : mrt::v3{0, 0, 0});
                put3(geom + 9 * i + 6, area ? l.tri.AC : mrt::v3{0, 0, 0});
            }
            if (coeffs != nullptr) putMaterial(coeffs + 13 * i, l.radiance);
        }
        n = static_cast<int64_t>(sc.lights.size());
    });
    return rc == 0 ? n : -1;
}

int64_t mrt_walk_tree(const mrt_config* cfg, uint32_t* nodes, float* grid, int32_t* root) {
    using namespace mrt;
    int64_t n = -1;
    const int rc = guarded([&] {
        HScene sc;
        const float ratio = cfg->height > 0 ? static_cast<float>(cfg->width) / static_cast<float>(cfg->height) : 1.0F;
        GCamera cam{};
        bool haveCam = true;
        if (cfg->sceneIndex >= 0 && cfg->sceneIndex <= 3) {
            sc = builtinScene(cfg->sceneIndex);
            cam = builtinCamera(cfg->sceneIndex, ratio);
        } else {
            std::string err;
            if (!loadObjScene(cfg->objFilePath ? cfg->objFilePath : "", cfg->mtlFilePath ? cfg->mtlFilePath : "", &sc,
                              &err))
                throw std::runtime_error(err);
            haveCam = loadCameraFile(cfg->camFilePath ? cfg->camFilePath : "", ratio, &cam, &err);
        }
        std::vector<int32_t> perm;
        const std::vector<HBVHNode> tn = buildBVH(&sc.triangles, &perm);
        GRoot r{};
        QGrid g{};
        std::vector<QNode4> qn;
        int top = 0;
        const int maxDepth = cfg->maxDepth > 0 ? cfg->maxDepth : kRayDepthMaxDefault;
        std::vector<double> cost;
        const std::vector<HBVHNode> wn = haveCam ? frameWalkTree(walkTreeOver(tn), sc, cam, cfg->width, cfg->height, maxDepth, &cost)
                                                 : walkTreeOver(tn);
        if (!toQuantizedBVH4(wn, sc.triangles.size(), &r, kTopNodesMax, &top, &g, &qn, nullptr,
                             cost.empty() ? nullptr : &cost))
            throw std::runtime_error("walk tree not quantizable (non-finite boxes)");
        n = static_cast<int64_t>(qn.size());
        if (nodes != nullptr) std::memcpy(nodes, qn.data(), qn.size() * sizeof(QNode4));
        if (grid != nullptr) {
            std::memcpy(grid, g.origin, sizeof(g.origin));
            std::memcpy(grid + 3, g.step, sizeof(g.step));
        }
        if (root != nullptr) {
            root[0] = r.ref;
            root[1] = r.count;
            root[2] = kWalkWidth;
        }
    });
    return rc == 0 ? n : -1;
}

int mrt_walk_stack(const mrt_config* cfg, int32_t* out) {
    using namespace mrt;
    return guarded([&] {
        HScene sc;
        const float ratio = cfg->height > 0 ? static_cast<float>(cfg->width) / static_cast<float>(cfg->height) : 1.0F;
        GCamera cam{};
        if (cfg->sceneIndex >= 0 && cfg->sceneIndex <= 3) {
            sc = builtinScene(cfg->sceneIndex);
            cam = builtinCamera(cfg->sceneIndex, ratio);
        } else {
            std::string err;
            if (!loadObjScene(cfg->objFilePath ? cfg->objFilePath : "", cfg->mtlFilePath ? cfg->mtlFilePath : "", &sc,
                              &err))
                throw std::runtime_error(err);
            if (!loadCameraFile(cfg->camFilePath ? cfg->camFilePath : "", ratio, &cam, &err)) throw std::runtime_error(err);
        }
        std::vector<int32_t> perm;
        const int otherDepth = std::max(bvhDepth(buildBVH(&sc.planes, &perm)), bvhDepth(buildBVH(&sc.spheres, &perm)));
        const std::vector<HBVHNode> tn = buildBVH(&sc.triangles, &perm);
        const int maxDepth = cfg->maxDepth > 0 ? cfg->maxDepth : kRayDepthMaxDefault;
        std::vector<double> cost;
        const std::vector<HBVHNode> wn = frameWalkTree(walkTreeOver(tn), sc, cam, cfg->width, cfg->height, maxDepth, &cost);
        GRoot root{};
        QGrid g{};
        std::vector<QNode4> qn;
        int top = 0;
        const bool quantized = toQuantizedBVH4(wn, sc.triangles.size(), &root, kTopNodesMax, &top, &g, &qn, nullptr,
                                               cost.empty() ? nullptr : &cost);
        const int depth4 = wideDepth(quantized, root, qn);
        out[0] = walkStackNeed(std::max({bvhDepth(tn), bvhDepth(wn), otherDepth}), depth4);
        out[1] = quantized ? 1 : 0;
        out[2] = bvhDepth(tn);
        out[3] = bvhDepth(wn);
        out[4] = depth4;
        out[5] = spillDepth(out[0]);
    });
}

int64_t mrt_plan_spill(int64_t threads, int32_t stackNeed, int64_t availBytes) {
    std::string err;
    const int64_t bytes = mrt::planSpillBytes(threads, spillDepth(stackNeed), availBytes, &err);
    if (bytes < 0) gLastError = err;
    return bytes;
}

int mrt_grid_box_test(int32_t kind, const float* prim, const float* box) {
    using namespace mrt;
    const HAABB b{v3{box[0], box[1], box[2]}, v3{box[3], box[4], box[5]}};
    const v3 p0{prim[0], prim[1], prim[2]}, p1{prim[3], prim[4], prim[5]};
    if (kind == 0) return boxIntersect(makeTriangle(p0, p1, v3{prim[6], prim[7], prim[8]}), b) ? 1 : 0;
    if (kind == 1) return boxIntersect(makePlane(p0, p1, -1), b) ? 1 : 0;
    if (kind == 2) return boxIntersect(makeSphere(p0, prim[3], -1), b) ? 1 : 0;
    gLastError = "grid box test: kind must be 0 (triangle), 1 (plane) or 2 (sphere)";
    return -1;
}

int64_t mrt_regular_grid(const mrt_config* cfg, int32_t kind, float* world, int32_t* start, int32_t* items) {
    using namespace mrt;
    int64_t n = -1;
    const int rc = guarded([&] {
        if (kind < 0 || kind > 2) throw std::runtime_error("regular grid: kind must be 0 (planes), 1 (spheres), 2 (triangles)");
        HScene sc;
        if (cfg->sceneIndex >= 0 && cfg->sceneIndex <= 3) {
            sc = builtinScene(cfg->sceneIndex);
        } else {
            std::string err;
            if (!loadObjScene(cfg->objFilePath ? cfg->objFilePath : "", cfg->mtlFilePath ? cfg->mtlFilePath : "", &sc,
                              &err))
                throw std::runtime_error(err);
        }
        std::vector<int32_t> order;
        HGrid g;
        if (kind == 0) {
            buildBVH(&sc.planes, &order);
            g = buildGrid(sc.planes, order);
        } else if (kind == 1) {
            buildBVH(&sc.spheres, &order);
            g = buildGrid(sc.spheres, order);
        } else {
            buildBVH(&sc.triangles, &order);
            g = buildGrid(sc.triangles, order);
        }
        n = static_cast<int64_t>(g.items.size());
        if (world != nullptr) {
            const float w[12] = {g.world.mn.x, g.world.mn.y, g.world.mn.z, g.world.mx.x, g.world.mx.y, g.world.mx.z,
                                 g.cellSize.x, g.cellSize.y, g.cellSize.z, g.cellSizeInv.x, g.cellSizeInv.y, g.cellSizeInv.z};
            std::memcpy(world, w, sizeof(w));
        }
        if (start != nullptr) std::memcpy(start, g.start.data(), g.start.size() * sizeof(int32_t));
        if (items != nullptr)
            for (size_t k = 0; k < g.items.size(); ++k) items[k] = order[static_cast<size_t>(g.items[k])];
    });
    return rc == 0 ? n : -1;
}

int64_t mrt_decode_texture(const char* path, int32_t* dims, uint8_t* texels) {
    int64_t n = -1;
    const int rc = guarded([&] {
        mrt::HTexture t;
        std::string err;
        if (!mrt::loadTextureFile(path != nullptr ? path : "", &t, &err)) throw std::runtime_error(err);
        n = static_cast<int64_t>(t.texels.size());
        if (dims != nullptr) {
            dims[0] = t.width;
            dims[1] = t.height;
            dims[2] = t.channels;
        }
        if (texels != nullptr) std::memcpy(texels, t.texels.data(), t.texels.size());
    });
    return rc == 0 ? n : -1;
}

int mrt_sample_tables(float* shader, float* sampler, float* trig) {
    return guarded([&] {
        std::vector<float> a, b, t;
        mrt::fillHaltonTable(&a, mrt::kSeedShaderTable);
        mrt::fillHaltonTable(&b, mrt::kSeedSamplerTable);
        mrt::fillHemisphereTrig(a, &t);
        if (shader != nullptr) std::memcpy(shader, a.data(), a.size() * sizeof(float));
        if (sampler != nullptr) std::memcpy(sampler, b.data(), b.size() * sizeof(float));
        if (trig != nullptr) std::memcpy(trig, t.data(), t.size() * sizeof(float));
    });
}

int mrt_get_tuning(const mrt_renderer* r, int32_t key, int32_t* value) {
    switch (key) {
        case 1: *value = r->ds.variant; return 0;
        case 2: *value = r->ds.cull; return 0;
        case 3: *value = r->overlap; return 0;
        case 7: *value = r->skipLast; return 0;
        case 5: *value = r->ds.anyOrder; return 0;
        case 6: *value = r->shadowGridPct; return 0;
        case 8: *value = r->ds.tailDonate; return 0;
        case 9: *value = r->refill; return 0;
        case 10: *value = r->ds.leanShade; return 0;
        case 11: *value = r->shadeGridPerCU; return 0;
        case 16: *value = r->ds.packet; return 0;
        case 17: *value = r->fuseL1Mode; return 0;
        case 27: *value = r->lastShadowRender; return 0;
        case 33: *value = r->genL1; return 0;
        case 34: *value = r->resolveAcc; return 0;
        case 35: *value = r->shadeWaitsShadow; return 0;
        case 28: *value = r->walkGridCap; return 0;
        case 37: *value = r->queueBudgetMiB; return 0;
        case 38: *value = r->queueGrowthPct; return 0;
        case 39: *value = r->queueSlack; return 0;
        case 40: *value = r->stackNeed; return 0;
        default: break;
    }
    gLastError = "unknown tuning key";
    return -1;
}

int mrt_get_frame_stats(const mrt_renderer* r, mrt_frame_stats* s) {
    *s = r->last;
    return 0;
}

int mrt_get_queue_info(const mrt_renderer* r, mrt_queue_info* out, size_t size) {
    using namespace mrt;
    if (r == nullptr || out == nullptr) {
        gLastError = "mrt_get_queue_info: null argument";
        return -1;
    }
    mrt_queue_info q{};
    q.chunkSlots = r->plan.chunkSlots;
    q.passes = (std::max<int64_t>(1, r->planSlots) + q.chunkSlots - 1) / std::max<int64_t>(1, q.chunkSlots);
    q.queueBytes = r->plan.bytes;
    q.budgetBytes = r->planBudget;
    q.replans = r->replans;
    q.replansLastFrame = r->replansFrame;
    q.worstCase = r->plan.worstCase;
    for (int l = 0; l < kMaxLevels && l < MRT_QUEUE_LEVELS; ++l) {
        q.rayCap[l] = l < r->nLevels ? r->plan.segCap[l] * kQueueSegs : 0;
        q.shadowCap[l] = l < r->nLevels ? r->plan.shadowSegCap[l] * kQueueSegs : 0;
        q.requestedRays[l] = r->reqRays[l];
        q.requestedShadows[l] = r->reqShadows[l];
    }
    for (const auto& p : r->peers) {
        q.queueBytes += p->plan.bytes;
        q.replans += p->replans;
        q.replansLastFrame += p->replansFrame;
        q.worstCase = std::max<int64_t>(q.worstCase, p->plan.worstCase);
    }
    std::memcpy(out, &q, std::min(size, sizeof(q)));
    return 0;
}

int mrt_plan_queues(const mrt_queue_plan_request* request, mrt_queue_plan* plan) {
    if (request == nullptr || plan == nullptr) {
        gLastError = "mrt_plan_queues: null argument";
        return -1;
    }
    std::string err;
    if (!mrt::planQueues(*request, plan, &err)) {
        gLastError = err;
        return -1;
    }
    return 0;
}

static void primaryHitsOne(mrt_renderer* r, int32_t* kind, int32_t* index, float* t);

int mrt_primary_hits(mrt_renderer* r, int32_t* kind, int32_t* index, float* t) {
    return guarded([&] {
        const size_t npx = static_cast<size_t>(r->cfg.width) * static_cast<size_t>(r->cfg.height);
        for (size_t i = 0; i < npx; ++i) {
            kind[i] = -1;
            index[i] = -1;
            t[i] = 0.0F;
        }
        for (int i = 0; i < groupSize(r); ++i) {
            mrt_renderer* p = shardOf(r, i);
            MRT_HIP(hipSetDevice(p->device));
            primaryHitsOne(p, kind, index, t);
        }
        MRT_HIP(hipSetDevice(r->device));
    });
}

static void primaryHitsOne(mrt_renderer* r, int32_t* kind, int32_t* index, float* t) {
    {
        using namespace mrt;
        hipStream_t st = r->stream;
        const auto& units = r->unitsByRank[static_cast<size_t>(r->rankIndex)];
        const auto& prefix = r->prefixByRank[static_cast<size_t>(r->rankIndex)];
        mrt_renderer::Pipe& pp = r->pipe;
        const int cap = pp.levels[1].cap;
        int32_t* dk = static_cast<int32_t*>(nullptr);
        int32_t* di = nullptr;
// ... 311 lines not shown
```

### mobileraytracer_amd/csrc/mrt_scene.cpp

```cpp
#include "mrt_scene.hpp"

#include <algorithm>
#include <limits>
#include <array>
#include <atomic>
#include <cmath>
#include <cstdlib>
#include <cstring>
#include <deque>
#include <functional>
#include <future>
#include <fstream>
#include <memory>
#include <mutex>
#include <queue>
#include <random>
#include <sstream>
#include <string>
#include <thread>
#include <unordered_map>

namespace mrt {

namespace {
// ... 969 lines not shown
        return dx * dy + dy * dz + dz * dx;
    };
    constexpr int W1 = kWalkWidth + 1;
    std::vector<double>& forest = *forestOut;
    std::vector<int8_t>& split = *splitOut;
    {
        forest.assign(nodes.size() * W1, 0.0);
        split.assign(nodes.size() * W1, 0);
        std::vector<std::pair<int32_t, bool>> post{{0, false}};
        while (!post.empty()) {
            const auto [i, done] = post.back();
            post.pop_back();
            if (!inner(i)) continue;
            const size_t ui = static_cast<size_t>(i);
            const int32_t l = nodes[ui].indexOffset, r = l + 1;
            if (!done) {
                post.push_back({i, true});
                post.push_back({l, false});
                post.push_back({r, false});
                continue;
            }
            const size_t ul = static_cast<size_t>(l) * W1, ur = static_cast<size_t>(r) * W1;
            auto best = [&](int j, int* k) {
                double c = std::numeric_limits<double>::infinity();
                for (int a = 1; a < j; ++a) {
                    const double v = forest[ul + static_cast<size_t>(a)] + forest[ur + static_cast<size_t>(j - a)];
                    if (v < c) {
                        c = v;
                        *k = a;
                    }
                }
                return c;
            };
            int kw = 1;
            const double asWide = area(i) + best(kWalkWidth, &kw);
            split[ui * W1] = static_cast<int8_t>(kw);
            forest[ui * W1 + 1] = asWide;
            for (int j = 2; j < W1; ++j) {
                int k = 1;
                const double c = best(j, &k);
                const bool self = asWide <= c;
                forest[ui * W1 + static_cast<size_t>(j)] = self ? asWide : c;
                split[ui * W1 + static_cast<size_t>(j)] = static_cast<int8_t>(self ? 0 : k);
            }
        }
    }
}

static double collapsedArea(const std::vector<HBVHNode>& nodes, int* depth) {
    *depth = 0;
    if (nodes.size() < 3 || nodes[0].numPrimitives > 0) return 0.0;
    std::vector<double> forest;
    std::vector<int8_t> split;
    collapseForests(nodes, &forest, &split);
    constexpr int W1 = kWalkWidth + 1;
    auto inner = [&](int32_t i) { return nodes[static_cast<size_t>(i)].numPrimitives == 0; };
    std::function<void(int32_t, int, std::vector<int32_t>&)> trees = [&](int32_t i, int j, std::vector<int32_t>& out) {
        const int k = inner(i) && j > 1 ? split[static_cast<size_t>(i) * W1 + static_cast<size_t>(j)] : 0;
        if (k == 0) {
            out.push_back(i);
            return;
        }
        trees(nodes[static_cast<size_t>(i)].indexOffset, k, out);
        trees(nodes[static_cast<size_t>(i)].indexOffset + 1, j - k, out);
    };
    std::vector<std::pair<int32_t, int>> st{{0, 1}};
    while (!st.empty()) {
        const auto [i, d] = st.back();
        st.pop_back();
        *depth = std::max(*depth, d);
        const int32_t l = nodes[static_cast<size_t>(i)].indexOffset;
        const int kw = split[static_cast<size_t>(i) * W1];
        std::vector<int32_t> c;
        trees(l, kw, c);
        trees(l + 1, kWalkWidth - kw, c);
        for (const int32_t k : c)
            if (inner(k)) st.push_back({k, d + 1});
    }
    return forest[1];
}

bool toQuantizedBVH4(const std::vector<HBVHNode>& nodes, size_t numPrims, GRoot* root, int topCount, int* topPlaced,
                     QGrid* grid, std::vector<QNode4>* out, std::vector<int32_t>* bvh2Of,
                     const std::vector<double>* nodeCost) {
    out->clear();
    if (bvh2Of != nullptr) bvh2Of->clear();
    if (topPlaced != nullptr) *topPlaced = 0;
    const HBVHNode& r = nodes[0];
    const float rmn[3] = {r.box.mn.x, r.box.mn.y, r.box.mn.z}, rmx[3] = {r.box.mx.x, r.box.mx.y, r.box.mx.z};
    for (int a = 0; a < 3; ++a) {
        root->bmin[a] = rmn[a];
        root->bmax[a] = rmx[a];
    }
    root->count = static_cast<int32_t>(numPrims);
    root->ref = 0;
    Quantizer qz;
    const bool gridOK = qz.init(rmn, rmx, grid);
    if (numPrims == 0) return gridOK;
    if (r.numPrimitives > 0) {
        root->ref = leafRef(r.indexOffset, r.numPrimitives);
        return gridOK;
    }
    if (!gridOK) return false;
    auto inner = [&](int32_t i) { return nodes[static_cast<size_t>(i)].numPrimitives == 0; };
    auto area = [&](int32_t i) {
        const HAABB& b = nodes[static_cast<size_t>(i)].box;
        const double dx = static_cast<double>(b.mx.x) - b.mn.x, dy = static_cast<double>(b.mx.y) - b.mn.y,
                     dz = static_cast<double>(b.mx.z) - b.mn.z;
        return dx * dy + dy * dz + dz * dx;
    };
    const char* collapseEnv = std::getenv("MOBILERT_COLLAPSE");
    const bool optimal = collapseEnv == nullptr || std::string(collapseEnv) != "greedy";
    constexpr int W1 = kWalkWidth + 1;
    std::vector<double> forest;
    std::vector<int8_t> split;
    if (optimal) collapseForests(nodes, &forest, &split, nodeCost);
    std::function<void(int32_t, int, std::vector<int32_t>&)> trees = [&](int32_t i, int j, std::vector<int32_t>& out) {
        const int k = inner(i) && j > 1 ? split[static_cast<size_t>(i) * W1 + static_cast<size_t>(j)] : 0;
        if (k == 0) {
            out.push_back(i);
            return;
        }
        trees(nodes[static_cast<size_t>(i)].indexOffset, k, out);
        trees(nodes[static_cast<size_t>(i)].indexOffset + 1, j - k, out);
    };
    std::vector<std::array<int32_t, kWalkWidth>> kids;
    std::vector<int32_t> node4Of(nodes.size(), -1);
    std::vector<int32_t> kidsBvh2{0};
    std::vector<int32_t> work{0};
    node4Of[0] = 0;
    kids.emplace_back();
    kids.back().fill(-1);
    while (!work.empty()) {
        const int32_t i = work.back();
        work.pop_back();
        const int32_t l = nodes[static_cast<size_t>(i)].indexOffset;
        std::vector<int32_t> c{l, l + 1};
        if (optimal) {
            const int kw = split[static_cast<size_t>(i) * W1];
            c.clear();
            trees(l, kw, c);
            trees(l + 1, kWalkWidth - kw, c);
        }
        while (!optimal && c.size() < static_cast<size_t>(kWalkWidth)) {
            int best = -1;
            double ba = -1.0;
            for (size_t k = 0; k < c.size(); ++k)
                if (inner(c[k]) && area(c[k]) > ba) {
                    ba = area(c[k]);
                    best = static_cast<int>(k);
                }
            if (best < 0) break;
            const int32_t cl = nodes[static_cast<size_t>(c[static_cast<size_t>(best)])].indexOffset;
            c[static_cast<size_t>(best)] = cl;
            c.insert(c.begin() + best + 1, cl + 1);
        }
        std::array<int32_t, kWalkWidth> k4;
        k4.fill(-1);
        for (size_t k = 0; k < c.size(); ++k) {
            k4[k] = c[k];
            if (inner(c[k])) {
                node4Of[static_cast<size_t>(c[k])] = static_cast<int32_t>(kids.size());
                kidsBvh2.push_back(c[k]);
                kids.emplace_back();
                kids.back().fill(-1);
                work.push_back(c[k]);
            }
        }
        kids[static_cast<size_t>(node4Of[static_cast<size_t>(i)])] = k4;
    }
    const size_t n4 = kids.size();
    std::vector<int32_t> newIdx(n4, -1), order;
    std::deque<int32_t> bfs{0};
    while (!bfs.empty() && static_cast<int>(order.size()) < topCount) {
        const int32_t j = bfs.front();
        bfs.pop_front();
        newIdx[static_cast<size_t>(j)] = static_cast<int32_t>(order.size());
        order.push_back(j);
        for (int32_t c : kids[static_cast<size_t>(j)])
            if (c >= 0 && inner(c)) bfs.push_back(node4Of[static_cast<size_t>(c)]);
    }
    if (topPlaced != nullptr) *topPlaced = static_cast<int>(order.size());
    std::vector<int32_t> dfs{0};
    while (!dfs.empty()) {
        const int32_t j = dfs.back();
        dfs.pop_back();
        if (newIdx[static_cast<size_t>(j)] < 0) {
            newIdx[static_cast<size_t>(j)] = static_cast<int32_t>(order.size());
            order.push_back(j);
        }
        const auto& k4 = kids[static_cast<size_t>(j)];
        for (int k = kWalkWidth - 1; k >= 0; --k)
            if (k4[static_cast<size_t>(k)] >= 0 && inner(k4[static_cast<size_t>(k)]))
                dfs.push_back(node4Of[static_cast<size_t>(k4[static_cast<size_t>(k)])]);
    }
    out->resize(n4);
    if (bvh2Of != nullptr) {
        bvh2Of->resize(n4);
        for (size_t k = 0; k < n4; ++k) (*bvh2Of)[k] = kidsBvh2[static_cast<size_t>(order[k])];
    }
    for (size_t k = 0; k < n4; ++k) {
        const auto& k4 = kids[static_cast<size_t>(order[k])];
        QNode4& q = (*out)[k];
        for (int c = 0; c < kWalkWidth; ++c) {
            const int32_t b = k4[static_cast<size_t>(c)];
            if (b < 0) {
                q.q[3 * c] = q.q[3 * c + 1] = q.q[3 * c + 2] = 0xFFFFu;
                q.ref[c] = kEmptyChild;
                continue;
            }
            const HBVHNode& bn = nodes[static_cast<size_t>(b)];
            const float mn[3] = {bn.box.mn.x, bn.box.mn.y, bn.box.mn.z}, mx[3] = {bn.box.mx.x, bn.box.mx.y, bn.box.mx.z};
            if (!qz.box(mn, mx, q.q + 3 * c)) {
                out->clear();
                return false;
            }
            q.ref[c] = bn.numPrimitives > 0 ? leafRef(bn.indexOffset, bn.numPrimitives)
                                             : newIdx[static_cast<size_t>(node4Of[static_cast<size_t>(b)])];
        }
    }
    root->ref = 0;
    return true;
}

namespace {
uint32_t coneWord(const std::vector<HTriangle>& tris, size_t lo, size_t hi) {
    double kMax = 1.0;
    double m[3][3] = {};
    std::vector<std::array<double, 3>> ns;
    ns.reserve(hi - lo);
    for (size_t i = lo; i < hi; ++i) {
        const HTriangle& t = tris[i];
        const double ab[3] = {t.AB.x, t.AB.y, t.AB.z}, ac[3] = {t.AC.x, t.AC.y, t.AC.z};
        const double n[3] = {ab[1] * ac[2] - ab[2] * ac[1], ab[2] * ac[0] - ab[0] * ac[2], ab[0] * ac[1] - ab[1] * ac[0]};
        const double len = std::sqrt(n[0] * n[0] + n[1] * n[1] + n[2] * n[2]);
        const double l1 = (std::fabs(ab[0]) + std::fabs(ab[1]) + std::fabs(ab[2])) *
                          (std::fabs(ac[0]) + std::fabs(ac[1]) + std::fabs(ac[2]));
        if (!(len > 0.0) || !std::isfinite(l1)) return kConeNever;
        kMax = std::max(kMax, l1 / len);
        const std::array<double, 3> u{n[0] / len, n[1] / len, n[2] / len};
        for (int r = 0; r < 3; ++r)
            for (int c = 0; c < 3; ++c) m[r][c] += u[static_cast<size_t>(r)] * u[static_cast<size_t>(c)];
        ns.push_back(u);
    }
    const double kCode = std::ceil(8.0 * std::log2(kMax) + 1e-9);
    if (ns.empty() || kCode > 126.0) return kConeNever;
    int col = 0;
    for (int c = 1; c < 3; ++c)
        if (m[c][c] > m[col][col]) col = c;
    double a[3] = {m[0][col], m[1][col], m[2][col]};
    for (int it = 0; it < 64; ++it) {
        double b[3];
        for (int r = 0; r < 3; ++r) b[r] = m[r][0] * a[0] + m[r][1] * a[1] + m[r][2] * a[2];
        const double l = std::sqrt(b[0] * b[0] + b[1] * b[1] + b[2] * b[2]);
        if (!(l > 0.0)) return kConeNever;
        for (int r = 0; r < 3; ++r) a[r] = b[r] / l;
    }
    const double s1 = std::fabs(a[0]) + std::fabs(a[1]) + std::fabs(a[2]);
    double ox = a[0] / s1, oy = a[1] / s1;
    if (a[2] < 0.0) {
        const double tx = ox;
        ox = (1.0 - std::fabs(oy)) * (tx >= 0.0 ? 1.0 : -1.0);
        oy = (1.0 - std::fabs(tx)) * (oy >= 0.0 ? 1.0 : -1.0);
    }
    const uint32_t qx = static_cast<uint32_t>(std::lround((ox + 1.0) * 0.5 * 511.0));
    const uint32_t qy = static_cast<uint32_t>(std::lround((oy + 1.0) * 0.5 * 511.0));
    const v3 dec = coneAxis(qx | (qy << 9));
    const double dl = std::sqrt(double(dec.x) * dec.x + double(dec.y) * dec.y + double(dec.z) * dec.z);
    const double ax[3] = {dec.x / dl, dec.y / dl, dec.z / dl};
    double cosMin = 1.0;
    for (const auto& u : ns) cosMin = std::min(cosMin, std::fabs(u[0] * ax[0] + u[1] * ax[1] + u[2] * ax[2]));
    const double psi = std::acos(std::min(1.0, cosMin)) + 2e-3;
    const double qCode = psi >= 1.5707963267948966 ? 127.0 : std::ceil(std::sin(psi) * 126.0 + 1e-9);
    if (qCode > 126.0) return kConeNever;
    return qx | (qy << 9) | (static_cast<uint32_t>(qCode) << 18) | (static_cast<uint32_t>(kCode) << 25);
}
}
// ... 477 lines not shown
    };
    auto closest = [&](v3 o, v3 d, float* tBest) {
        const v3 inv{1.0F / d.x, 1.0F / d.y, 1.0F / d.z};
        int best = -1;
        float bt = std::numeric_limits<float>::infinity();
        std::vector<int32_t> st{0};
        while (!st.empty()) {
            const size_t i = static_cast<size_t>(st.back());
            st.pop_back();
            if (!(entry(nodes[i].box, o, inv) < bt)) continue;
            if (inner(i)) {
                st.push_back(nodes[i].indexOffset + 1);
                st.push_back(nodes[i].indexOffset);
                continue;
            }
            for (int32_t k = 0; k < nodes[i].numPrimitives; ++k) {
                float t;
                const int32_t j = nodes[i].indexOffset + k;
                if (triHit(sc.triangles[static_cast<size_t>(j)], o, d, &t) && t < bt) {
                    bt = t;
                    best = j;
                }
            }
        }
        for (const HLight& l : sc.lights) {
            float t;
            if (l.kind == kAreaLight && triHit(l.tri, o, d, &t) && t < bt) {
                bt = t;
                best = -2;
            }
        }
        *tBest = bt;
        return best;
    };
    std::vector<const HLight*> areaLights;
    for (const HLight& l : sc.lights)
        if (l.kind == kAreaLight) areaLights.push_back(&l);
    std::mt19937 rng(0x4D525406u);
    std::uniform_real_distribution<float> U(0.0F, 1.0F);
    constexpr float camW = 0.6F, shadowW = 1.0F;
    constexpr int gx = 192, gy = 108;
    struct Path {
        v3 o, d;
        int depth;
    };
    for (int py = 0; py < gy; ++py)
        for (int px = 0; px < gx; ++px) {
            const float u = (static_cast<float>(px) + U(rng)) / static_cast<float>(gx);
            const float v = (static_cast<float>(py) + U(rng)) / static_cast<float>(gy);
            v3 o, d;
            if (cam.kind == 1) {
                o = (cam.position + cam.right * ((u - 0.5F) * cam.hFov)) + cam.up * ((0.5F - v) * cam.vFov);
                d = cam.direction;
            } else {
                const v3 dest = ((cam.position + cam.direction) + cam.right * fastArcTan(cam.hFov * (u - 0.5F))) +
                                cam.up * fastArcTan(cam.vFov * (0.5F - v));
                o = cam.position;
                d = normalize(dest - cam.position);
            }
            std::vector<Path> work{{o, d, 1}};
            while (!work.empty()) {
                const Path p = work.back();
                work.pop_back();
                rays.push_back(Ray{p.o, p.d, p.depth == 1 ? camW : 1.0F});
                float t;
                const int hit = closest(p.o, p.d, &t);
                if (hit < 0) continue;
                const HTriangle& tri = sc.triangles[static_cast<size_t>(hit)];
                const HMaterial m = tri.mat >= 0 && tri.mat < static_cast<int32_t>(sc.materials.size())
                                        ? sc.materials[static_cast<size_t>(tri.mat)] : HMaterial{};
                if (m.Le.x > 0.0F || m.Le.y > 0.0F || m.Le.z > 0.0F) continue;
                v3 n = normalize(cross(tri.AB, tri.AC));
                if (dot(n, p.d) > 0.0F) n = -n;
                const v3 P = p.o + p.d * t + n * 1e-3F;
                const bool diffuse = m.Kd.x > 0.0F || m.Kd.y > 0.0F || m.Kd.z > 0.0F;
                if (diffuse && !areaLights.empty()) {
                    const HLight& l = *areaLights[static_cast<size_t>(U(rng) * 0.99999F * static_cast<float>(areaLights.size()))];
                    float r1 = U(rng), r2 = U(rng);
                    if (r1 + r2 >= 1.0F) {
                        r1 = 1.0F - r1;
                        r2 = 1.0F - r2;
                    }
                    const v3 q = (l.tri.A + l.tri.AB * r1) + l.tri.AC * r2;
                    rays.push_back(Ray{P, normalize(q - P), shadowW});
                }
                if (p.depth >= maxDepth) continue;
                if (diffuse && (p.depth <= 1 || U(rng) > 0.5F)) {
                    const float phi = 6.2831853F * U(rng), r2 = U(rng);
                    const v3 a = std::fabs(n.x) > 0.1F ? v3{0.0F, 1.0F, 0.0F} : v3{1.0F, 0.0F, 0.0F};
                    const v3 tu = normalize(cross(a, n)), tv = cross(n, tu);
                    const float ct = std::sqrt(r2);
                    work.push_back(Path{P, normalize((tu * (std::cos(phi) * ct) + tv * (std::sin(phi) * ct)) + n * std::sqrt(1.0F - r2)),
                                        p.depth + 1});
                }
                if (m.Ks.x > 0.0F || m.Ks.y > 0.0F || m.Ks.z > 0.0F) work.push_back(Path{P, reflect(p.d, n), p.depth + 1});
            }
        }
    return rays;
}

std::vector<double> frameRayNodeCosts(const std::vector<HBVHNode>& nodes, const HScene& sc, const GCamera& cam,
                                      int width, int height, int maxDepth) {
    if (nodes.empty() || sc.triangles.empty() || width <= 0 || height <= 0) return std::vector<double>(nodes.size(), 0.0);
    return sampleRayNodeCosts(nodes, sampleFrameRays(nodes, sc, cam, maxDepth));
}

constexpr float kRayCostFloor = 0.01F;

std::vector<double> sampleRayNodeCosts(const std::vector<HBVHNode>& nodes, const std::vector<SampleRay>& rays) {
    std::vector<double> cost(nodes.size(), 0.0);
    if (nodes.empty() || rays.empty()) return cost;
    auto inner = [&](size_t i) { return nodes[i].numPrimitives == 0 && nodes.size() > 1; };
    constexpr float floorW = kRayCostFloor;
    const unsigned hw = std::max(1u, std::min(16u, std::thread::hardware_concurrency()));
    std::vector<std::vector<double>> part(hw, std::vector<double>(nodes.size(), 0.0));
    std::vector<std::thread> pool;
    for (unsigned w = 0; w < hw; ++w)
        pool.emplace_back([&, w] {
            std::vector<int32_t> st;
            std::vector<double>& c = part[w];
            for (size_t k = w; k < rays.size(); k += hw) {
                const SampleRay& r = rays[k];
                const v3 inv{1.0F / r.d.x, 1.0F / r.d.y, 1.0F / r.d.z};
                st.assign(1, 0);
                while (!st.empty()) {
                    const size_t i = static_cast<size_t>(st.back());
                    st.pop_back();
                    if (!(halfLineEntry(nodes[i].box, r.o, inv) < std::numeric_limits<float>::infinity())) continue;
                    c[i] += r.w;
                    if (inner(i)) {
                        st.push_back(nodes[i].indexOffset);
                        st.push_back(nodes[i].indexOffset + 1);
                    }
                }
            }
        });
    for (std::thread& t : pool) t.join();
    double total = 0.0;
    for (const SampleRay& r : rays) total += r.w;
    auto area = [&](size_t i) {
        const HAABB& b = nodes[i].box;
        const double dx = static_cast<double>(b.mx.x) - b.mn.x, dy = static_cast<double>(b.mx.y) - b.mn.y,
                     dz = static_cast<double>(b.mx.z) - b.mn.z;
        return dx * dy + dy * dz + dz * dx;
    };
    const double rootArea = std::max(1e-30, area(0));
    for (size_t i = 0; i < nodes.size(); ++i) {
        double s = 0.0;
        for (unsigned w = 0; w < hw; ++w) s += part[w][i];
        cost[i] = s + floorW * total * area(i) / rootArea;
    }
    return cost;
}

std::vector<HBVHNode> rotateForRays(const std::vector<HBVHNode>& in, const std::vector<SampleRay>& rays, int sweeps) {
    if (in.size() < 8 || sweeps <= 0 || rays.empty() || in[0].numPrimitives > 0) return in;
    constexpr int W1 = kWalkWidth + 1;
    struct R {
        HAABB box;
        int32_t l = -1, r = -1, parent = -1, first = 0, count = 0;
        int32_t height = 0, maxHeight = 0;
        double cost = 0.0;
        double F[W1] = {};
    };
    std::vector<R> t;
    {
        std::vector<std::pair<int32_t, int32_t>> st{{0, -1}};
        while (!st.empty()) {
            const auto [i, parent] = st.back();
            st.pop_back();
            const int32_t k = static_cast<int32_t>(t.size());
            t.emplace_back();
            R& n = t.back();
            const HBVHNode& h = in[static_cast<size_t>(i)];
            n.box = h.box;
            n.parent = parent;
            if (parent >= 0) {
                R& pn = t[static_cast<size_t>(parent)];
                (pn.l < 0 ? pn.l : pn.r) = k;
            }
            if (h.numPrimitives > 0) {
                n.first = h.indexOffset;
                n.count = h.numPrimitives;
            } else {
                st.push_back({h.indexOffset + 1, k});
                st.push_back({h.indexOffset, k});
            }
        }
    }
    const size_t nn = t.size();
    auto inner = [&](int32_t i) { return t[static_cast<size_t>(i)].count == 0; };
    for (size_t k = nn; k-- > 0;) {
        R& n = t[k];
        if (n.count == 0)
            n.height = 1 + std::max(t[static_cast<size_t>(n.l)].height, t[static_cast<size_t>(n.r)].height);
        n.maxHeight = n.height;
    }
    auto area = [](const HAABB& b) {
        const double dx = static_cast<double>(b.mx.x) - b.mn.x, dy = static_cast<double>(b.mx.y) - b.mn.y,
                     dz = static_cast<double>(b.mx.z) - b.mn.z;
        return dx * dy + dy * dz + dz * dx;
    };
    double total = 0.0;
    for (const SampleRay& ry : rays) total += ry.w;
    const double rootArea = std::max(1e-30, area(t[0].box));
    const double floorK = kRayCostFloor * total / rootArea;
    std::vector<v3> inv(rays.size());
    for (size_t k = 0; k < rays.size(); ++k) inv[k] = v3{1.0F / rays[k].d.x, 1.0F / rays[k].d.y, 1.0F / rays[k].d.z};
    auto passes = [&](const HAABB& b, int32_t k) {
        return halfLineEntry(b, rays[static_cast<size_t>(k)].o, inv[static_cast<size_t>(k)]) < std::numeric_limits<float>::infinity();
    };
    std::vector<std::vector<int32_t>> list(nn);
    {
        const unsigned hw = std::max(1u, std::min(16u, std::thread::hardware_concurrency()));
        std::vector<std::vector<std::vector<int32_t>>> part(hw);
        std::vector<std::thread> pool;
        for (unsigned w = 0; w < hw; ++w)
            pool.emplace_back([&, w] {
                std::vector<std::vector<int32_t>>& pl = part[w];
                pl.assign(nn, {});
                std::vector<int32_t> st;
                for (size_t k = w; k < rays.size(); k += hw) {
                    st.assign(1, 0);
                    while (!st.empty()) {
                        const int32_t i = st.back();
                        st.pop_back();
                        const R& n = t[static_cast<size_t>(i)];
                        if (n.count > 0 || !passes(n.box, static_cast<int32_t>(k))) continue;
                        pl[static_cast<size_t>(i)].push_back(static_cast<int32_t>(k));
                        st.push_back(n.l);
                        st.push_back(n.r);
                    }
                }
// ... 252 lines not shown
```

### mobileraytracer_amd/csrc/mrt_scene.hpp

```cpp
#pragma once

#include "mrt_common.hpp"

#include <functional>
#include <istream>
#include <string>
#include <array>
#include <vector>

namespace mrt {

struct v2 {
    float x, y;
};

struct HMaterial {
    v3 Le{0, 0, 0}, Kd{0, 0, 0}, Ks{0, 0, 0}, Kt{0, 0, 0};
    float ior{1.0F};
    std::string texture;
    int32_t texId{-1};
};

struct HTexture {
    int32_t width{0}, height{0}, channels{0};
    std::vector<uint8_t> texels;
};
bool decodePng(const std::vector<uint8_t>& file, HTexture* out, std::string* err);
bool loadTextureFile(const std::string& path, HTexture* out, std::string* err);
bool materialEqual(const HMaterial& a, const HMaterial& b);

struct HTriangle {
    v3 AC, AB, A;
    v3 nA, nB, nC;
    v2 tA{-1, -1}, tB{-1, -1}, tC{-1, -1};
    int32_t mat{-1};
};
HTriangle makeTriangle(v3 a, v3 b, v3 c);
HTriangle makeTriangle(v3 a, v3 b, v3 c, v3 na, v3 nb, v3 nc, v2 ta, v2 tb, v2 tc, int32_t mat);

struct HPlane {
    v3 normal, point;
    int32_t mat;
};
HPlane makePlane(v3 point, v3 normal, int32_t mat);

struct HSphere {
    v3 center;
    float sqRadius;
    int32_t mat;
};
HSphere makeSphere(v3 center, float radius, int32_t mat);

enum LightKind : int32_t { kPointLight = 0, kAreaLight = 1 };
struct HLight {
    int32_t kind;
    HMaterial radiance;
    v3 position;
    HTriangle tri;
};

struct HAABB {
    v3 mn, mx;
};

struct HScene {
    std::vector<HPlane> planes;
    std::vector<HSphere> spheres;
    std::vector<HTriangle> triangles;
    std::vector<HLight> lights;
    std::vector<HMaterial> materials;
    std::vector<HTexture> textures;
};

struct HBVHNode {
    HAABB box;
    int32_t indexOffset;
    int32_t numPrimitives;
};

HScene cornellBoxScene();
HScene builtinScene(int index);
GCamera builtinCamera(int index, float ratio);
v3 builtinMaxPoint(int index);
GCamera makeOrthographic(v3 position, v3 lookAt, v3 up, float sizeH, float sizeV);
GCamera cornellBoxCamera(float ratio);
GCamera makePerspective(v3 position, v3 lookAt, v3 up, float hFovDeg, float vFovDeg);
bool loadCameraFile(const std::string& path, float ratio, GCamera* out, std::string* err);
bool loadCameraStream(std::istream& in, float ratio, GCamera* out, std::string* err, const std::string& name = "");
bool loadObjScene(const std::string& objPath, const std::string& mtlPath, HScene* scene, std::string* err);
using TextureSource = std::function<bool(const std::string&, HTexture*)>;
bool loadObjStreams(std::istream& obj, std::istream* mtl, const TextureSource& textureSource, HScene* scene,
                    std::string* err);

template <class It, class Pred>
It pinnedPartition(It first, It last, Pred pred) {
    while (true) {
        while (true) {
            if (first == last) return first;
            if (pred(*first)) ++first; else break;
        }
        --last;
        while (true) {
            if (first == last) return first;
            if (!pred(*last)) --last; else break;
        }
        auto tmp = *first;
        *first = *last;
        *last = tmp;
        ++first;
    }
}

HAABB aabbOf(const HTriangle& t);
HAABB aabbOf(const HPlane& p);
HAABB aabbOf(const HSphere& s);
bool aabbIntersect(const HAABB& b, v3 origin, v3 dir);

template <class T>
std::vector<HBVHNode> buildBVH(std::vector<T>* prims, std::vector<int32_t>* order);

void toDeviceBVH(const std::vector<HBVHNode>& nodes, size_t numPrims, std::vector<GNode>* out, GRoot* root,
                 int topCount = 0, int* topPlaced = nullptr, const std::vector<uint32_t>* cones = nullptr);
bool toQuantizedBVH4(const std::vector<HBVHNode>& nodes, size_t numPrims, GRoot* root, int topCount, int* topPlaced,
                     QGrid* grid, std::vector<QNode4>* out, std::vector<int32_t>* bvh2Of = nullptr,
                     const std::vector<double>* nodeCost = nullptr);
std::vector<double> frameRayNodeCosts(const std::vector<HBVHNode>& nodes, const HScene& sc, const GCamera& cam,
                                      int width, int height, int maxDepth);
struct SampleRay {
    v3 o, d;
    float w;
};
std::vector<SampleRay> sampleFrameRays(const std::vector<HBVHNode>& nodes, const HScene& sc, const GCamera& cam,
                                       int maxDepth);
std::vector<double> sampleRayNodeCosts(const std::vector<HBVHNode>& nodes, const std::vector<SampleRay>& rays);
std::vector<HBVHNode> rotateForRays(const std::vector<HBVHNode>& in, const std::vector<SampleRay>& rays, int sweeps);
std::vector<HBVHNode> rebuildOverLeaves(const std::vector<HBVHNode>& ref, int weight = 0);
std::vector<HBVHNode> optimizeOverLeaves(const std::vector<HBVHNode>& tree, int rounds, bool bounded = true);
constexpr int kTreeOptRounds = 100;
constexpr int kTreeRotSweeps = 1;
constexpr size_t kTreeCacheScenes = 4;
std::vector<HBVHNode> walkTreeOver(const std::vector<HBVHNode>& ref);
std::vector<uint32_t> triangleConeWords(const std::vector<HBVHNode>& nodes, const std::vector<HTriangle>& tris);
void leafCullRecord(const std::vector<HTriangle>& tris, size_t lo, size_t hi, const HAABB& box, float out[6]);
void cullRecord(const std::vector<HTriangle>& tris, const std::vector<std::array<int32_t, 2>>& ranges,
                const double ctr[3], double hd, float out[6]);

struct HGrid {
    HAABB world;
    v3 cellSize, cellSizeInv;
    int32_t count = 0;
    std::vector<int32_t> start, items;
};
bool boxIntersect(const HTriangle& t, const HAABB& box);
bool boxIntersect(const HPlane& p, const HAABB& box);
bool boxIntersect(const HSphere& s, const HAABB& box);
template <class T>
HGrid buildGrid(const std::vector<T>& prims, const std::vector<int32_t>& order);

float haltonSequence(uint32_t index, uint32_t base);
void fillHaltonTable(std::vector<float>* table, uint32_t seed);
void fillHemisphereTrig(const std::vector<float>& shaderTable, std::vector<float>* out);
constexpr uint32_t kSeedShaderTable = 0x4D525400u;
constexpr uint32_t kSeedSamplerTable = 0x4D525401u;

std::vector<int32_t> parseDeviceList(const char* s);

}
```

### mobileraytracer_amd/csrc/mrt_trace_ww.hpp

```cpp
#pragma once

#include "mrt_device.hpp"
#include "mrt_kernels.hpp"

namespace mrt {

constexpr int kRefDone = 0x7FFFFFFF;
constexpr int kWalkRefill = 32;
constexpr int kWalkShards = kMaxFetchShards;
#ifndef MRT_WALK_SEGMENTS
#define MRT_WALK_SEGMENTS 2
#endif
__device__ __forceinline__ int walkSegments() {
    return gridDim.x >= static_cast<unsigned>(kWalkShards) ? MRT_WALK_SEGMENTS : kWalkShards;
}
constexpr int kWalkStack = kLdsStackMin;
constexpr int kWalkTop = kTopNodesMax;
#ifndef MRT_INNER_EXIT
#define MRT_INNER_EXIT 4
#endif
#ifndef MRT_INNER_EXIT_ANY
#define MRT_INNER_EXIT_ANY MRT_INNER_EXIT
#endif
constexpr int kInnerExitClosest = MRT_INNER_EXIT;
// ... 194 lines not shown
    const float tMax = fminf(fminf(fx, fy), fz);
    *tEntry = e;
    return tMax >= e;
}

__device__ __forceinline__ void cex(float& ka, int& ra, float& kb, int& rb) {
    const bool sw = kb < ka;
    const float k = sw ? kb : ka;
    const int r = sw ? rb : ra;
    kb = sw ? ka : kb;
    rb = sw ? ra : rb;
    ka = k;
    ra = r;
}

template <int W>
__device__ __forceinline__ void sortChildren(float* k, int* r) {
    if (W == 4) {
        cex(k[0], r[0], k[1], r[1]);
        cex(k[2], r[2], k[3], r[3]);
        cex(k[0], r[0], k[2], r[2]);
        cex(k[1], r[1], k[3], r[3]);
        cex(k[1], r[1], k[2], r[2]);
    } else {
        constexpr int net[19][2] = {{0, 1}, {2, 3}, {4, 5}, {6, 7}, {0, 2}, {1, 3}, {4, 6}, {5, 7}, {1, 2}, {5, 6},
                                    {0, 4}, {1, 5}, {2, 6}, {3, 7}, {2, 4}, {3, 5}, {1, 2}, {3, 4}, {5, 6}};
#pragma unroll
        for (int c = 0; c < 19; ++c) cex(k[net[c][0]], r[net[c][0]], k[net[c][1]], r[net[c][1]]);
    }
}

template <int kCull, int kOrder, class Stack>
__device__ __forceinline__ int innerStepQ(BufRes qnodes, const QNode4* ldsTop, int top, int ref, v3 qa, v3 qb,
                                          float lim, Stack& st, TravCount* cnt, bool count) {
    constexpr int W = kWalkWidth;
    constexpr bool cull = kCull != kCullNone;
    int4 raw[W];
    if (ref < top) {
        const int4* np = reinterpret_cast<const int4*>(ldsTop + ref);
#pragma unroll
        for (int j = 0; j < W; ++j) raw[j] = np[j];
    } else {
        const uint32_t off = static_cast<uint32_t>(ref) * static_cast<uint32_t>(sizeof(QNode4));
#pragma unroll
        for (int j = 0; j < W; ++j) raw[j] = bload4i(qnodes, off + 16u * static_cast<uint32_t>(j));
    }
    const auto word = [&](int i) -> uint32_t {
        const int4 v = raw[i >> 2];
        const int c = i & 3;
        return static_cast<uint32_t>(c == 0 ? v.x : c == 1 ? v.y : c == 2 ? v.z : v.w);
    };
    constexpr float kInf = __builtin_inff();
    const uint32_t sx = nearFarShift(qa.x), sy = nearFarShift(qa.y), sz = nearFarShift(qa.z);
    constexpr float sg = kOrder == 0 ? 1.0F : -1.0F;
    float key[W];
    int rf[W];
    int n = 0;
#pragma unroll
    for (int c = 0; c < W; ++c) {
        const uint32_t w0 = word(3 * c), w1 = word(3 * c + 1), w2 = word(3 * c + 2);
        rf[c] = static_cast<int>(word(3 * W + c));
        if (count) cnt->nodes += rf[c] != kEmptyChild ? 1u : 0u;
        float t;
        bool h = qslabNF(w0, w1, w2, sx, sy, sz, qa, qb, &t);
        if (cull) h = h && !(t > lim);
        n += h ? 1 : 0;
        key[c] = h ? sg * t : kInf;
    }
    if (n == 0) return popCulled(st, lim, cull);
    sortChildren<W>(key, rf);
#pragma unroll
    for (int k = W - 1; k >= 1; --k)
        if (k < n) st.push(rf[k], sg * key[k]);
    return rf[0];
}

__device__ __forceinline__ bool quantOK(const DScene& s, v3 o, v3 inv) {
    if (s.qEnabled == 0) return false;
    const float ov[3] = {o.x, o.y, o.z}, iv[3] = {inv.x, inv.y, inv.z};
    bool ok = true;
#pragma unroll
    for (int a = 0; a < 3; ++a) {
        const float ai = fabsf(iv[a]);
        ok = ok && ai >= 0x1p-40F && ai <= 0x1p90F && ai * s.qgrid.step[a] >= 0x1p-100F &&
             fabsf(ov[a] - s.qgrid.origin[a]) <= 4.0F * 65535.0F * s.qgrid.step[a];
    }
    return ok;
}

template <int kThreads>
__device__ __forceinline__ void stageTop(const DScene& s, QNode4* ldsTop) {
    const int n = min(kWalkTop, s.triTop) * static_cast<int>(sizeof(QNode4) / sizeof(float4));
    const float4* src = reinterpret_cast<const float4*>(s.triQNodes);
    float4* dst = reinterpret_cast<float4*>(ldsTop);
    for (int i = static_cast<int>(threadIdx.x); i < n; i += kThreads) dst[i] = src[i];
    __syncthreads();
}

#ifndef MRT_SEG_INTERLEAVE
#define MRT_SEG_INTERLEAVE 1
#endif
#ifndef MRT_TRI_PREFETCH
#define MRT_TRI_PREFETCH 1
#endif
#ifndef MRT_TRI_PREFETCH_ANY
#define MRT_TRI_PREFETCH_ANY MRT_TRI_PREFETCH
#endif
#ifndef MRT_SEG_REVERSE
#define MRT_SEG_REVERSE 1
#endif
#ifndef MRT_TRI_SPREAD
#define MRT_TRI_SPREAD 1
#endif
#ifndef MRT_TRI_SPREAD_ANY
#define MRT_TRI_SPREAD_ANY MRT_TRI_SPREAD
#endif
#ifndef MRT_SEG_CHUNK_LOG
#define MRT_SEG_CHUNK_LOG 12
#endif
constexpr int kSegChunkLog = MRT_SEG_CHUNK_LOG;
__device__ __forceinline__ int segChunkShift(int n, int maxLog) {
    const int per = max(n >> 6, 1);
    return min(maxLog, 31 - __clz(per));
}
__device__ __forceinline__ int interleavedIndex(int j, int seg, int shift) {
    return ((((j >> shift) * kWalkShards) + seg) << shift) + (j & ((1 << shift) - 1));
}

static_assert(kQueueSegs == 1 || kWalkShards % kQueueSegs == 0, "queue segments: whole cursors each");
struct LevelQueue {
    const float4* __restrict__ rO;
    const float4* __restrict__ rD;
    float4* out;
    SegMap map;
    int count;
    int* fetch;
    int seg = static_cast<int>(blockIdx.x % kWalkShards);
    int segsLeft = walkSegments();
    int shift;
    __device__ __forceinline__ LevelQueue(const float4* o_, const float4* d_, float4* out_, const SegMap& map_, int* fetch_)
        : rO(o_), rD(d_), out(out_), map(map_), count(map_.total()), fetch(fetch_),
          shift(segChunkShift(map_.total(), kSegChunkLog)) {}
    __device__ __forceinline__ int segCount(int g) const {
        int c = 0;
#pragma unroll
        for (int k = 0; k < kQueueSegs; ++k)
            if (k == g) c = map.pre[k + 1] - map.pre[k];
        return c;
    }
    __device__ __forceinline__ float4 o(int i) const { return rO[i]; }
    __device__ __forceinline__ float4 d(int i) const { return rD[i]; }
    __device__ __forceinline__ void hit(int i, float4 h) const { out[i] = h; }
    __device__ __forceinline__ void occ(int i, float f) const { out[i].w = f; }
    __device__ __forceinline__ bool drained() const { return segsLeft == 0; }
    __device__ __forceinline__ int take(uint64_t pending) {
        const int lane = static_cast<int>(threadIdx.x & 63u);
        int got = -1;
        while (pending != 0 && segsLeft > 0) {
            const int n = __popcll(pending);
            const int leader = __ffsll(static_cast<unsigned long long>(pending)) - 1;
            const int segStart = static_cast<int>((static_cast<long long>(count) * seg) / kWalkShards);
            const int segEnd = static_cast<int>((static_cast<long long>(count) * (seg + 1)) / kWalkShards);
            int base = 0;
            if (lane == leader) base = atomicAdd(fetch + seg * kFetchStride, n);
            base = __shfl(base, leader, 64);
            const bool mine = ((pending >> lane) & 1ull) != 0;
            if (kQueueSegs > 1) {
                (void)segStart;
                (void)segEnd;
                constexpr int kParts = kWalkShards / kQueueSegs;
                const int g = seg % kQueueSegs, part = seg / kQueueSegs;
                const int cnt = segCount(g);
                const int lo = static_cast<int>((static_cast<long long>(cnt) * part) / kParts);
                const int hi = static_cast<int>((static_cast<long long>(cnt) * (part + 1)) / kParts);
                const int idx = base + lanesBelowIn(pending);
                if (mine && idx < hi - lo) got = g * map.segCap + (hi - 1 - idx);
            } else if (mine) {
#if MRT_SEG_INTERLEAVE
                (void)segStart;
                (void)segEnd;
                const int idx = interleavedIndex(base + lanesBelowIn(pending), seg, shift);
#if MRT_SEG_REVERSE
                if (idx < count) got = count - 1 - idx;
#else
                if (idx < count) got = idx;
#endif
#else
                const int idx = segStart + base + lanesBelowIn(pending);
                if (idx < segEnd) got = idx;
#endif
            }
            pending = __ballot(mine && got < 0);
            if (pending != 0) {
                seg = (seg + 1) % kWalkShards;
                --segsLeft;
            }
        }
        return got;
    }
};

template <bool kAny, bool kCount, int kCull, class Stack, class Queue>
__device__ __forceinline__ void traceWhileWhileQ(const DScene& s, Queue& q, Stack& st, TravCount* cnt,
                                                 const QNode4* ldsTop, int* tailBest) {
    constexpr int kSpread = kAny ? MRT_TRI_SPREAD_ANY : MRT_TRI_SPREAD;
    __shared__ uint8_t spreadOwners[kSpread != 0 ? 192 * 4 : 1];
    constexpr int kHelper = -2;
    const bool donate = s.tailDonate != 0;
    const int top = min(kWalkTop, s.triTop);
    const BufRes nodeBuf = bufferOf(s.triNodes);
    const BufRes qBuf = bufferOf(s.triQNodes);
    const BufRes triBuf = bufferOf(s.triGeom);
    const BufRes leafBuf = bufferOf(s.leafBoxes);
    constexpr int kInner = innerCullMode<kCull>();
    constexpr bool cull = kInner != kCullNone;
    const int lane = static_cast<int>(threadIdx.x & 63u);
    int rayIdx = -1;
    bool exhausted = false;
    v3 o{0, 0, 0}, d{0, 0, 0}, inv{0, 0, 0};
    v3 qa{0, 0, 0}, qb{0, 0, 0};
    bool refTree = true;
    uint32_t src = 0;
    float bt = kRayLengthMax;
    uint32_t bcode = kNoPrim;
    int ref = kRefDone;
    int leaf = 0;
    int owner = -1;
    int pend = 0;
    bool occ = false;
    bool tailMode = false;
    float shT = __builtin_inff();
    int* const waveBest = tailBest + (threadIdx.x & ~63u);
    while (true) {
        if (tailMode && rayIdx != -1) {
            const int ol = rayIdx >= 0 ? lane : owner;
            const int mine = kAny ? (occ ? 0 : 0x7FFFFFFF) : __float_as_int(bt);
            const int v = min(atomicMin(waveBest + ol, mine), mine);
            if (kAny) {
                if (v == 0 && !occ) {
                    occ = rayIdx >= 0;
                    st.sp = 0;
                    ref = kRefDone;
                    leaf = 0;
                }
            } else {
                shT = __int_as_float(v);
            }
        }
        const bool over = ref == kRefDone && leaf >= 0;
        if (donate) {
            uint64_t hm = __ballot(rayIdx == kHelper && over);
            while (hm != 0) {
                const int h = __ffsll(static_cast<unsigned long long>(hm)) - 1;
                hm &= hm - 1;
                const int ol = __builtin_amdgcn_readlane(owner, h);
                const float ht = __int_as_float(__builtin_amdgcn_readlane(__float_as_int(bt), h));
                const uint32_t hc = static_cast<uint32_t>(__builtin_amdgcn_readlane(static_cast<int>(bcode), h));
                const int ho = __builtin_amdgcn_readlane(occ ? 1 : 0, h);
                if (lane == ol) {
                    if (kAny) {
                        occ = occ || ho != 0;
                    } else if (betterThan(ht, hc, bt, bcode)) {
                        bt = ht;
                        bcode = hc;
                    }
                    --pend;
                }
            }
            if (rayIdx == kHelper && over) {
                rayIdx = -1;
                occ = false;
            }
        }
        const bool doneLane = rayIdx >= 0 && over && pend == 0;
        bool runDone = true;
        if (!kAny) {
            const int nReady = __popcll(__ballot(doneLane || (rayIdx == -1 && !exhausted)));
            runDone = nReady >= s.refill || __ballot(rayIdx >= 0 && !doneLane) == 0 || __ballot(exhausted) != 0;
        }
        if (doneLane && runDone) {
            if (kCount) cnt->rayMax = max(cnt->rayMax, cnt->nodes - cnt->rayStart);
            if (kAny) {
                q.occ(rayIdx, occ ? 1.0F : 0.0F);
                if (kCount) cnt->occluded += occ ? 1u : 0u;
                occ = false;
            } else {
                for (int j = 0; j < s.nLights; ++j) {
                    const float4* l = s.lights + 4 * j;
                    const float4 a4 = l[0];
// ... 157 lines not shown
        const uint32_t doneLanes = kCount ? static_cast<uint32_t>(__popcll(__ballot(rayIdx != -1 && over2(ref, leaf)))) : 0u;
        const v3 qaL = kSpread == 0 ? qa : v3{s.qgrid.step[0] * inv.x, s.qgrid.step[1] * inv.y, s.qgrid.step[2] * inv.z};
        const v3 qbL = kSpread == 0 ? qb : v3{(s.qgrid.origin[0] - o.x) * inv.x, (s.qgrid.origin[1] - o.y) * inv.y,
                                              (s.qgrid.origin[2] - o.z) * inv.z};
        while (static_cast<unsigned>(ref) < static_cast<unsigned>(kRefDone)) {
            if (kCount) {
                phaseCount(&cnt->innerIters, &cnt->innerLanes);
                if (lanesBelowIn(__ballot(true)) == 0) {
                    cnt->innerIdle += idleLanes;
                    cnt->innerDone += doneLanes;
                }
            }
            const float curLim = cullLimit<kInner>(fminf(bt, shT));
            const bool finite = __ballot(!finiteInv(inv)) == 0;
            const int order = kAny ? s.anyOrder : 0;
            ref = refTree ? innerStep<kInner>(nodeBuf, ref, o, d, inv, curLim, st, cnt, kCount, finite, order)
                          : order == 0 ? innerStepQ<kInner, 0>(qBuf, ldsTop, top, ref, qaL, qbL, curLim, st, cnt, kCount)
                                       : innerStepQ<kInner, 1>(qBuf, ldsTop, top, ref, qaL, qbL, curLim, st, cnt, kCount);
            if (ref < 0 && leaf >= 0) {
                leaf = ref;
                ref = popCulled(st, curLim, cull);
            }
            if (__popcll(__ballot(leaf >= 0 && static_cast<unsigned>(ref) < static_cast<unsigned>(kRefDone))) < innerExit)
                break;
        }
        if constexpr (kSpread != 0) {
        constexpr uint32_t kNoHitBits = 0x7F800001u;
        while (__ballot(leaf < 0) != 0) {
            const bool holding = leaf < 0;
            int first = 0, nprim = 0;
            float4 a0 = make_float4(0.0F, 0.0F, 0.0F, 0.0F), b0t = a0, c0 = a0;
            if (holding) {
                if (kCount) phaseCount(&cnt->leafIters, &cnt->leafLanes);
                first = leafFirst(leaf);
                nprim = leafCount(leaf);
                const uint32_t off0 = static_cast<uint32_t>(first) * 48u;
                a0 = bload3(triBuf, off0);
                b0t = bload3(triBuf, off0 + 16u);
                c0 = bload3(triBuf, off0 + 32u);
                if (!refTree) {
                    const uint32_t lo = static_cast<uint32_t>(first) * 48u;
                    const float4 b0 = bload4(leafBuf, lo);
                    if (kCount) ++cnt->leaves;
                    if (kCull == kCullExact) {
                        const float4 b1 = bload4(leafBuf, lo + 16u);
                        const float4 b2 = bload4(leafBuf, lo + 32u);
                        float te, ex, ey, ez;
                        if (!slabFiniteAxes(b0.x, b0.y, b0.z, b0.w, b1.x, b1.y, o, inv, &te, &ex, &ey, &ez)) {
                            nprim = 0;
                        } else {
                            const float lim = fminf(bt, shT);
                            if (te > lim && leafKey(b1, b2, te, ex, ey, ez, d, inv) > lim) nprim = 0;
                        }
                    } else {
                        const int2 b1 = bload2i(leafBuf, lo + 16u);
                        float te;
                        const bool in =
                            slabFinite(b0.x, b0.y, b0.z, b0.w, __int_as_float(b1.x), __int_as_float(b1.y), o, inv, &te);
                        if (!in || (cull && te > cullLimit<kCull>(fminf(bt, shT)))) nprim = 0;
                    }
                }
            }
            bool hit = false;
            if (nprim > 0) {
                if (kCount) phaseCount(&cnt->triIters, &cnt->triLanes);
                const uint32_t code = encodePrim(kTriangle, static_cast<uint32_t>(first));
                float t, u, v;
                if (code != src) {
                    if (kCount) ++cnt->tris;
                    if (triTest(a0, b0t, c0, o, d, &t, &u, &v) && !(t < kEpsilon)) {
                        if (kAny) {
                            hit = !(t >= bt);
                        } else if (betterThan(t, code, bt, bcode)) {
                            bt = t;
                            bcode = code;
                        }
                    }
                }
            }
            const uint64_t m1 = __ballot(nprim > 1 && !hit);
            if (m1 != 0) {
                const uint64_t m2 = __ballot(nprim > 2 && !hit), m3 = __ballot(nprim > 3 && !hit);
                const int c1 = __popcll(m1), c12 = c1 + __popcll(m2), total = c12 + __popcll(m3);
                uint8_t* const owners = spreadOwners + 192 * (threadIdx.x >> 6);
                if (nprim > 1 && !hit) owners[lanesBelowIn(m1)] = static_cast<uint8_t>(lane);
                if (nprim > 2 && !hit) owners[c1 + lanesBelowIn(m2)] = static_cast<uint8_t>(lane);
                if (nprim > 3 && !hit) owners[c12 + lanesBelowIn(m3)] = static_cast<uint8_t>(lane);
                __builtin_amdgcn_wave_barrier();
                bool hit2 = false;
                for (int base = 0; base < total; base += 64) {
                    const int g = base + lane;
                    const int tk = g < c1 ? 1 : g < c12 ? 2 : 3;
                    const int own = g < total ? static_cast<int>(owners[g]) : lane;
                    const int srcLane = own << 2;
                    const v3 to{__int_as_float(__builtin_amdgcn_ds_bpermute(srcLane, __float_as_int(o.x))),
                                __int_as_float(__builtin_amdgcn_ds_bpermute(srcLane, __float_as_int(o.y))),
                                __int_as_float(__builtin_amdgcn_ds_bpermute(srcLane, __float_as_int(o.z)))};
                    const v3 td{__int_as_float(__builtin_amdgcn_ds_bpermute(srcLane, __float_as_int(d.x))),
                                __int_as_float(__builtin_amdgcn_ds_bpermute(srcLane, __float_as_int(d.y))),
                                __int_as_float(__builtin_amdgcn_ds_bpermute(srcLane, __float_as_int(d.z)))};
                    const uint32_t tsrc = static_cast<uint32_t>(__builtin_amdgcn_ds_bpermute(srcLane, static_cast<int>(src)));
                    const int tj = leafFirst(__builtin_amdgcn_ds_bpermute(srcLane, leaf)) + tk;
                    uint32_t tt = kNoHitBits;
                    if (g < total) {
                        if (kCount) phaseCount(&cnt->triIters, &cnt->triLanes);
                        const uint32_t code = encodePrim(kTriangle, static_cast<uint32_t>(tj));
                        if (code != tsrc) {
                            if (kCount) ++cnt->tris;
                            const uint32_t off = static_cast<uint32_t>(tj) * 48u;
                            const float4 ta = bload3(triBuf, off), tb = bload3(triBuf, off + 16u), tc = bload3(triBuf, off + 32u);
                            float t, u, v;
                            if (triTest(ta, tb, tc, to, td, &t, &u, &v) && !(t < kEpsilon)) tt = __float_as_uint(t);
                        }
                    }
#pragma unroll
                    for (int k = 1; k <= 3; ++k) {
                        const uint64_t mk = k == 1 ? m1 : k == 2 ? m2 : m3;
                        const int idx = (k == 1 ? 0 : k == 2 ? c1 : c12) + lanesBelowIn(mk);
                        const bool mine = ((mk >> lane) & 1ull) != 0 && idx >= base && idx < base + 64;
                        const uint32_t rt = static_cast<uint32_t>(__builtin_amdgcn_ds_bpermute((idx - base) << 2, static_cast<int>(tt)));
                        if (mine && rt != kNoHitBits) {
                            const float t = __uint_as_float(rt);
                            const uint32_t code = encodePrim(kTriangle, static_cast<uint32_t>(leafFirst(leaf) + k));
                            if (kAny) {
                                hit2 = hit2 || !(t >= bt);
                            } else if (betterThan(t, code, bt, bcode)) {
                                bt = t;
                                bcode = code;
                            }
                        }
                    }
                }
                hit = hit || hit2;
                __builtin_amdgcn_wave_barrier();
            }
            if (holding) {
                if (kAny && hit) {
                    if (kCount) cnt->occluded += (rayIdx >= 0 && pend == 0) ? 1u : 0u;
                    if (rayIdx >= 0 && pend == 0) {
                        q.occ(rayIdx, 1.0F);
                        rayIdx = -1;
                    } else {
                        occ = true;
                    }
                    st.sp = 0;
                    ref = kRefDone;
                    leaf = 0;
                } else {
                    leaf = 0;
                    if (ref < 0) {
                        leaf = ref;
                        ref = popCulled(st, cullLimit<kInner>(fminf(bt, shT)), cull);
                    }
                }
            }
            if (__popcll(__ballot(leaf < 0)) < leafExit) break;
        }
        } else {
        while (leaf < 0) {
            if (kCount) phaseCount(&cnt->leafIters, &cnt->leafLanes);
            const int first = leafFirst(leaf);
            int nprim = leafCount(leaf);
            const uint32_t off0 = static_cast<uint32_t>(first) * 48u;
            const float4 a0 = bload3(triBuf, off0), b0t = bload3(triBuf, off0 + 16u), c0 = bload3(triBuf, off0 + 32u);
            if (!refTree) {
                const uint32_t lo = static_cast<uint32_t>(first) * 48u;
                const float4 b0 = bload4(leafBuf, lo);
// ... 90 lines not shown
```

Baseline: 5397 Mrays/s.

## Size LDS top-of-tree cache to fill budget and pick hottest nodes by visits

The number of BVH4 nodes cached in LDS for the per-lane walk is no longer a fixed 64 nodes. It is now computed from an LDS budget per workgroup that still allows six groups (24 waves) per CU. Which nodes go into that cache is chosen by sampled ray visit counts, with each shadow sample ray limited to its light distance, instead of breadth-first order. This is meant to cut global memory fetches of frequently visited inner nodes, at the cost of more LDS per block and a hot set that could miss rays unlike the samples. It also adds a diagnostic API, runtime tuning keys, and a scalarised bound check.

```diff
diff --git a/__graft_entry__.py b/__graft_entry__.py
--- a/__graft_entry__.py
+++ b/__graft_entry__.py
@@ -12,6 +12,7 @@
     subprocess.run(["make", "-j", jobs, "-C", os.path.join(HERE, "mobileraytracer_amd", "csrc")], check=True)
     subprocess.run(["make", "-C", os.path.join(HERE, "oracle")], check=True)
     subprocess.run(["make", "-C", os.path.join(HERE, "tests", "cabi")], check=True)
+    subprocess.run(["make", "-C", os.path.join(HERE, "tests", "hosttop")], check=True)
     from mobileraytracer_amd import scenes
     scenes.conference()
     scenes.conference_flat()
diff --git a/include/mobilert_amd.h b/include/mobilert_amd.h
--- a/include/mobilert_amd.h
+++ b/include/mobilert_amd.h
@@ -177,6 +177,7 @@
 int64_t mrt_triangle_bvh(const mrt_config *cfg, float *boxes, int32_t *offsets, int32_t *counts, int32_t *order);
 int64_t mrt_walk_tree(const mrt_config *cfg, uint32_t *nodes, float *grid, int32_t *root);
 int mrt_walk_stack(const mrt_config *cfg, int32_t *out);
+int64_t mrt_walk_top(const mrt_config *cfg, int32_t *info, double *share, double *visits);
 int64_t mrt_plan_spill(int64_t threads, int32_t stackNeed, int64_t availBytes);
 int64_t mrt_regular_grid(const mrt_config *cfg, int32_t kind, float *world, int32_t *start, int32_t *items);
 int mrt_grid_box_test(int32_t kind, const float *prim, const float *box);
diff --git a/mobileraytracer_amd/__init__.py b/mobileraytracer_amd/__init__.py
--- a/mobileraytracer_amd/__init__.py
+++ b/mobileraytracer_amd/__init__.py
@@ -413,6 +413,22 @@
     _native.check(_native.lib().mrt_walk_stack(ctypes.byref(c), _ptr(out)))
     return {"need": int(out[0]), "quantized": bool(out[1]), "refDepth": int(out[2]), "walkDepth": int(out[3]),
             "wideDepth": int(out[4]), "spillDepth": int(out[5])}
+
+
+def walk_top(config: Config) -> dict:
+    lib = _native.lib()
+    c = config.to_c()
+    info = np.zeros(4, np.int32)
+    share = np.zeros(3, np.float64)
+    n = lib.mrt_walk_top(ctypes.byref(c), _ptr(info), _ptr(share), None)
+    if n < 0:
+        raise RuntimeError(lib.mrt_last_error().decode())
+    visits = np.zeros(n, np.float64)
+    if n > 0 and lib.mrt_walk_top(ctypes.byref(c), None, None, _ptr(visits)) != n:
+        raise RuntimeError(lib.mrt_last_error().decode())
+    return {"capacity": int(info[0]), "staged": int(info[1]), "nodes": int(info[2]), "hotFirst": bool(info[3]),
+            "totalVisits": float(share[0]), "share": float(share[1]), "shareBreadthFirst": float(share[2]),
+            "visits": visits}
 
 
 def plan_spill(threads: int, stack_need: int, avail_bytes: int = 0) -> int:
diff --git a/mobileraytracer_amd/_native.py b/mobileraytracer_amd/_native.py
--- a/mobileraytracer_amd/_native.py
+++ b/mobileraytracer_amd/_native.py
@@ -20,7 +20,7 @@
     "mrt_kat_accumulate", "mrt_cast_rays_device", "mrt_walk_stack", "mrt_plan_spill",
     "mrt_path_key", "mrt_shade_rays_device", "mrt_camera_rays_device",
     "mrt_cast_hits_device", "mrt_scene_triangles", "mrt_scene_planes", "mrt_scene_spheres", "mrt_scene_materials",
-    "mrt_scene_lights",
+    "mrt_scene_lights", "mrt_walk_top",
     "RayTrace", "stopRender",
 )
 
@@ -171,6 +171,7 @@
         "mrt_triangle_bvh": (ctypes.c_int64, [vp, vp, vp, vp, vp]),
         "mrt_walk_tree": (ctypes.c_int64, [vp, vp, vp, vp]),
         "mrt_walk_stack": (ctypes.c_int, [vp, vp]),
+        "mrt_walk_top": (ctypes.c_int64, [vp, vp, vp, vp]),
         "mrt_plan_spill": (ctypes.c_int64, [ctypes.c_int64, ctypes.c_int32, ctypes.c_int64]),
         "mrt_decode_texture": (ctypes.c_int64, [ctypes.c_char_p, vp, vp]),
         "mrt_regular_grid": (ctypes.c_int64, [vp, ctypes.c_int32, vp, vp, vp]),
diff --git a/mobileraytracer_amd/csrc/mrt_kernels.hip b/mobileraytracer_amd/csrc/mrt_kernels.hip
--- a/mobileraytracer_amd/csrc/mrt_kernels.hip
+++ b/mobileraytracer_amd/csrc/mrt_kernels.hip
@@ -157,7 +157,6 @@
     lv.tree[p] = 1u;
 }
 
-constexpr int kWalkThreads = 256;
 
 template <bool kCount>
 __device__ __forceinline__ void reduceCounts(const TravCount& cnt, unsigned long long* stats, int nodesStat,
@@ -199,7 +198,7 @@
         n += __shfl_down(n, off, 64);
         r += __shfl_down(r, off, 64);
     }
-    const int wave = static_cast<int>(blockIdx.x * (kWalkThreads / 64) + threadIdx.x / 64);
+    const int wave = static_cast<int>(blockIdx.x * kWalkWaves + threadIdx.x / 64);
     if (laneId() == 0 && wave < kWaveLogWaves && level < kMaxLevels) {
         unsigned long long* e = stats + kNumStats + ((static_cast<size_t>(kind) * kMaxLevels + level) * kWaveLogWaves + wave) * 4;
         e[0] = t0;
diff --git a/mobileraytracer_amd/csrc/mrt_kernels.hpp b/mobileraytracer_amd/csrc/mrt_kernels.hpp
--- a/mobileraytracer_amd/csrc/mrt_kernels.hpp
+++ b/mobileraytracer_amd/csrc/mrt_kernels.hpp
@@ -15,7 +15,19 @@
 constexpr int kAccNaive = 1;
 constexpr int kAccGrid = 2;
 constexpr int kAccBVH = 3;
-constexpr int kTopNodesMax = 64 * 4 / kWalkWidth;
+constexpr int kWalkThreads = 256;
+constexpr int kWalkWaves = kWalkThreads / 64;
+constexpr int kLaneWalkGroupsPerCU = 6;
+constexpr int kSpreadOwnersPerWave = 192;
+constexpr int kLaneWalkLdsPerGroup = (160 * 1024 / kLaneWalkGroupsPerCU) / 1280 * 1280;
+constexpr int kLaneWalkLdsFixed = kWalkThreads * (8 * kLdsStackMin + 4) + kWalkWaves * kSpreadOwnersPerWave;
+#ifdef MRT_TOP_NODES
+constexpr int kTopNodesMax = MRT_TOP_NODES;
+#else
+constexpr int kTopNodesMax = (kLaneWalkLdsPerGroup - kLaneWalkLdsFixed) / static_cast<int>(sizeof(QNode4));
+#endif
+static_assert(kTopNodesMax >= 0 && kTopNodesMax * static_cast<int>(sizeof(QNode4)) + kLaneWalkLdsFixed <= kLaneWalkLdsPerGroup,
+              "the LDS top must leave the per-lane walks their 24 waves per CU");
 
 #ifndef MRT_QUEUE_SEGS
 #define MRT_QUEUE_SEGS 8
diff --git a/mobileraytracer_amd/csrc/mrt_renderer.hip b/mobileraytracer_amd/csrc/mrt_renderer.hip
--- a/mobileraytracer_amd/csrc/mrt_renderer.hip
+++ b/mobileraytracer_amd/csrc/mrt_renderer.hip
@@ -70,6 +70,7 @@
 struct FrameTree {
     std::vector<mrt::HBVHNode> nodes;
     std::vector<double> cost;
+    std::vector<double> visits;
 };
 struct Fnv64 {
     uint64_t h = 1469598103934665603ull;
@@ -81,8 +82,10 @@
     void pod(const T& v) { add(&v, sizeof(v)); }
 };
 std::vector<mrt::HBVHNode> frameWalkTree(const std::vector<mrt::HBVHNode>& wn, const mrt::HScene& sc, const mrt::GCamera& cam,
-                                         int width, int height, int maxDepth, std::vector<double>* cost) {
+                                         int width, int height, int maxDepth, std::vector<double>* cost,
+                                         std::vector<double>* visits) {
     cost->clear();
+    visits->clear();
     const char* ce = std::getenv("MOBILERT_COLLAPSE");
     if (ce != nullptr && (std::string(ce) == "area" || std::string(ce) == "greedy")) return wn;
     if (wn.empty() || sc.triangles.empty() || width <= 0 || height <= 0) {
@@ -136,15 +139,17 @@
     if (pending.valid()) {
         const Entry e = pending.get();
         *cost = e->cost;
+        *visits = e->visits;
         return e->nodes;
     }
     try {
         auto e = std::make_shared<FrameTree>();
         const std::vector<mrt::SampleRay> rays = mrt::sampleFrameRays(wn, sc, cam, maxDepth);
         e->nodes = sweeps > 0 ? mrt::rotateForRays(wn, rays, sweeps) : wn;
-        e->cost = mrt::sampleRayNodeCosts(e->nodes, rays);
+        e->cost = mrt::sampleRayNodeCosts(e->nodes, rays, &e->visits);
         mine.set_value(e);
         *cost = e->cost;
+        *visits = e->visits;
         return e->nodes;
     } catch (...) {
         mine.set_exception(std::current_exception());
@@ -153,6 +158,22 @@
         order.erase(std::remove(order.begin(), order.end(), f.h), order.end());
         throw;
     }
+}
+
+int topNodesWanted() {
+    const char* e = std::getenv("MOBILERT_TOP_NODES");
+    if (e == nullptr || *e == '\0') return mrt::kTopNodesMax;
+    return std::max(0, std::min(mrt::kTopNodesMax, std::atoi(e)));
+}
+bool topHotFirst() {
+    const char* e = std::getenv("MOBILERT_TOP_ORDER");
+    return e == nullptr || std::string(e) != "bfs";
+}
+bool quantizedWalkTree(const std::vector<mrt::HBVHNode>& wn, size_t numPrims, const std::vector<double>& cost,
+                       const std::vector<double>& visits, mrt::GRoot* root, int* top, mrt::QGrid* grid,
+                       std::vector<mrt::QNode4>* qn, std::vector<double>* wideVisits = nullptr, bool breadthFirst = false) {
+    return mrt::toQuantizedBVH4(wn, numPrims, root, topNodesWanted(), top, grid, qn, nullptr, cost.empty() ? nullptr : &cost,
+                                visits.empty() ? nullptr : &visits, wideVisits, topHotFirst() && !breadthFirst);
 }
 
 int bvhDepth(const std::vector<mrt::HBVHNode>& nodes) {
@@ -355,6 +376,7 @@
     int64_t reqPaths = 0;
     int gdepth = 0;
     int traceThreads = 0, workGrid = 0;
+    int triTopPlaced = 0, triTopCap = -1;
     int cus = 0;
     int shadeGridPerCU = -1;
     int32_t* dBitmap = nullptr;
@@ -506,9 +528,9 @@
     std::vector<HBVHNode> pn = buildBVH(&sc.planes, &r->planeOrder);
     std::vector<HBVHNode> sn = buildBVH(&sc.spheres, &r->sphereOrder);
     std::vector<HBVHNode> tn = buildBVH(&sc.triangles, &r->triOrder);
-    std::vector<double> rayCost;
+    std::vector<double> rayCost, rayVisits;
     const std::vector<HBVHNode> wn =
-        frameWalkTree(walkTreeOver(tn), sc, r->cam, r->cfg.width, r->cfg.height, r->maxDepth, &rayCost);
+        frameWalkTree(walkTreeOver(tn), sc, r->cam, r->cfg.width, r->cfg.height, r->maxDepth, &rayCost, &rayVisits);
     r->nTri = static_cast<int64_t>(sc.triangles.size());
     r->nPlanes = static_cast<int64_t>(sc.planes.size());
     r->nSpheres = static_cast<int64_t>(sc.spheres.size());
@@ -526,9 +548,13 @@
     DScene& d = r->ds;
     const std::vector<uint32_t> conesRef = triangleConeWords(tn, sc.triangles);
     std::vector<QNode4> qn;
-    d.qEnabled = toQuantizedBVH4(wn, sc.triangles.size(), &d.triRoot, kTopNodesMax, &d.triTop, &d.qgrid, &qn, nullptr,
-                                 rayCost.empty() ? nullptr : &rayCost) ? 1 : 0;
-    if (d.qEnabled == 0 || qn.empty()) qn.resize(1);
+    d.qEnabled = quantizedWalkTree(wn, sc.triangles.size(), rayCost, rayVisits, &d.triRoot, &d.triTop, &d.qgrid, &qn) ? 1 : 0;
+    if (d.qEnabled == 0 || qn.empty()) {
+        qn.resize(1);
+        d.triTop = 0;
+    }
+    r->triTopPlaced = d.triTop;
+    if (r->triTopCap >= 0) d.triTop = std::min(d.triTop, r->triTopCap);
     d.triQNodes = r->sceneMem.upload(qn, st);
     {
         static_assert(kWalkWidth == 4, "packet nodes: 4 children");
@@ -2138,6 +2164,11 @@
         r->planStale = true;
         return 0;
     }
+    if (key == 41 && value >= -1 && value <= mrt::kTopNodesMax) {
+        r->triTopCap = value;
+        r->ds.triTop = value < 0 ? r->triTopPlaced : std::min(r->triTopPlaced, value);
+        return 0;
+    }
     gLastError = "unknown tuning key/value";
     return -1;
 }
@@ -2288,11 +2319,10 @@
         std::vector<QNode4> qn;
         int top = 0;
         const int maxDepth = cfg->maxDepth > 0 ? cfg->maxDepth : kRayDepthMaxDefault;
-        std::vector<double> cost;
-        const std::vector<HBVHNode> wn = haveCam ? frameWalkTree(walkTreeOver(tn), sc, cam, cfg->width, cfg->height, maxDepth, &cost)
+        std::vector<double> cost, visits;
+        const std::vector<HBVHNode> wn = haveCam ? frameWalkTree(walkTreeOver(tn), sc, cam, cfg->width, cfg->height, maxDepth, &cost, &visits)
                                                  : walkTreeOver(tn);
-        if (!toQuantizedBVH4(wn, sc.triangles.size(), &r, kTopNodesMax, &top, &g, &qn, nullptr,
-                             cost.empty() ? nullptr : &cost))
+        if (!quantizedWalkTree(wn, sc.triangles.size(), cost, visits, &r, &top, &g, &qn))
             throw std::runtime_error("walk tree not quantizable (non-finite boxes)");
         n = static_cast<int64_t>(qn.size());
         if (nodes != nullptr) std::memcpy(nodes, qn.data(), qn.size() * sizeof(QNode4));
@@ -2329,14 +2359,13 @@
         const int otherDepth = std::max(bvhDepth(buildBVH(&sc.planes, &perm)), bvhDepth(buildBVH(&sc.spheres, &perm)));
         const std::vector<HBVHNode> tn = buildBVH(&sc.triangles, &perm);
         const int maxDepth = cfg->maxDepth > 0 ? cfg->maxDepth : kRayDepthMaxDefault;
-        std::vector<double> cost;
-        const std::vector<HBVHNode> wn = frameWalkTree(walkTreeOver(tn), sc, cam, cfg->width, cfg->height, maxDepth, &cost);
+        std::vector<double> cost, visits;
+        const std::vector<HBVHNode> wn = frameWalkTree(walkTreeOver(tn), sc, cam, cfg->width, cfg->height, maxDepth, &cost, &visits);
         GRoot root{};
         QGrid g{};
         std::vector<QNode4> qn;
         int top = 0;
-        const bool quantized = toQuantizedBVH4(wn, sc.triangles.size(), &root, kTopNodesMax, &top, &g, &qn, nullptr,
-                                               cost.empty() ? nullptr : &cost);
+        const bool quantized = quantizedWalkTree(wn, sc.triangles.size(), cost, visits, &root, &top, &g, &qn);
         const int depth4 = wideDepth(quantized, root, qn);
         out[0] = walkStackNeed(std::max({bvhDepth(tn), bvhDepth(wn), otherDepth}), depth4);
         out[1] = quantized ? 1 : 0;
@@ -2345,6 +2374,61 @@
         out[4] = depth4;
         out[5] = spillDepth(out[0]);
     });
+}
+
+int64_t mrt_walk_top(const mrt_config* cfg, int32_t* info, double* share, double* visits) {
+    using namespace mrt;
+    int64_t n = -1;
+    const int rc = guarded([&] {
+        HScene sc;
+        const float ratio = cfg->height > 0 ? static_cast<float>(cfg->width) / static_cast<float>(cfg->height) : 1.0F;
+        GCamera cam{};
+        bool haveCam = true;
+        if (cfg->sceneIndex >= 0 && cfg->sceneIndex <= 3) {
+            sc = builtinScene(cfg->sceneIndex);
+            cam = builtinCamera(cfg->sceneIndex, ratio);
+        } else {
+            std::string err;
+            if (!loadObjScene(cfg->objFilePath ? cfg->objFilePath : "", cfg->mtlFilePath ? cfg->mtlFilePath : "", &sc,
+                              &err))
+                throw std::runtime_error(err);
+            haveCam = loadCameraFile(cfg->camFilePath ? cfg->camFilePath : "", ratio, &cam, &err);
+        }
+        std::vector<int32_t> perm;
+        const std::vector<HBVHNode> tn = buildBVH(&sc.triangles, &perm);
+        const int maxDepth = cfg->maxDepth > 0 ? cfg->maxDepth : kRayDepthMaxDefault;
+        std::vector<double> cost, nodeVisits;
+        const std::vector<HBVHNode> wn = haveCam ? frameWalkTree(walkTreeOver(tn), sc, cam, cfg->width, cfg->height, maxDepth, &cost, &nodeVisits)
+                                                 : walkTreeOver(tn);
+        GRoot r{};
+        QGrid g{};
+        std::vector<QNode4> qn;
+        std::vector<double> shipped, bfs;
+        int top = 0, topBfs = 0;
+        const bool quantized = quantizedWalkTree(wn, sc.triangles.size(), cost, nodeVisits, &r, &top, &g, &qn, &shipped);
+        quantizedWalkTree(wn, sc.triangles.size(), cost, nodeVisits, &r, &topBfs, &g, &qn, &bfs, true);
+        n = quantized ? static_cast<int64_t>(qn.size()) : 0;
+        const auto sum = [](const std::vector<double>& v, size_t k) {
+            double s = 0.0;
+            for (size_t i = 0; i < std::min(k, v.size()); ++i) s += v[i];
+            return s;
+        };
+        const double total = sum(shipped, shipped.size());
+        if (info != nullptr) {
+            info[0] = topNodesWanted();
+            info[1] = quantized ? top : 0;
+            info[2] = static_cast<int32_t>(n);
+            info[3] = topHotFirst() && !nodeVisits.empty() ? 1 : 0;
+        }
+        if (share != nullptr) {
+            share[0] = total;
+            share[1] = total > 0.0 ? sum(shipped, static_cast<size_t>(top)) / total : 0.0;
+            share[2] = total > 0.0 ? sum(bfs, static_cast<size_t>(topBfs)) / total : 0.0;
+        }
+        if (visits != nullptr)
+            for (int64_t k = 0; k < n; ++k) visits[k] = static_cast<size_t>(k) < shipped.size() ? shipped[static_cast<size_t>(k)] : 0.0;
+    });
+    return rc == 0 ? n : -1;
 }
 
 int64_t mrt_plan_spill(int64_t threads, int32_t stackNeed, int64_t availBytes) {
@@ -2456,6 +2540,8 @@
         case 38: *value = r->queueGrowthPct; return 0;
         case 39: *value = r->queueSlack; return 0;
         case 40: *value = r->stackNeed; return 0;
+        case 41: *value = r->ds.triTop; return 0;
+        case 42: *value = mrt::kTopNodesMax; return 0;
         default: break;
     }
     gLastError = "unknown tuning key";
diff --git a/mobileraytracer_amd/csrc/mrt_scene.cpp b/mobileraytracer_amd/csrc/mrt_scene.cpp
--- a/mobileraytracer_amd/csrc/mrt_scene.cpp
+++ b/mobileraytracer_amd/csrc/mrt_scene.cpp
@@ -1075,9 +1075,11 @@
 
 bool toQuantizedBVH4(const std::vector<HBVHNode>& nodes, size_t numPrims, GRoot* root, int topCount, int* topPlaced,
                      QGrid* grid, std::vector<QNode4>* out, std::vector<int32_t>* bvh2Of,
-                     const std::vector<double>* nodeCost) {
+                     const std::vector<double>* nodeCost, const std::vector<double>* nodeVisits,
+                     std::vector<double>* wideVisits, bool hotFirstTop) {
     out->clear();
     if (bvh2Of != nullptr) bvh2Of->clear();
+    if (wideVisits != nullptr) wideVisits->clear();
     if (topPlaced != nullptr) *topPlaced = 0;
     const HBVHNode& r = nodes[0];
     const float rmn[3] = {r.box.mn.x, r.box.mn.y, r.box.mn.z}, rmx[3] = {r.box.mx.x, r.box.mx.y, r.box.mx.z};
@@ -1163,29 +1165,61 @@
         kids[static_cast<size_t>(node4Of[static_cast<size_t>(i)])] = k4;
     }
     const size_t n4 = kids.size();
-    std::vector<int32_t> newIdx(n4, -1), order;
+    std::vector<int32_t> newIdx, order;
+    const auto number = [&](const std::vector<int32_t>& first) {
+        newIdx.assign(n4, -1);
+        order.clear();
+        for (const int32_t j : first) {
+            newIdx[static_cast<size_t>(j)] = static_cast<int32_t>(order.size());
+            order.push_back(j);
+        }
+        std::vector<int32_t> dfs{0};
+        while (!dfs.empty()) {
+            const int32_t j = dfs.back();
+            dfs.pop_back();
+            if (newIdx[static_cast<size_t>(j)] < 0) {
+                newIdx[static_cast<size_t>(j)] = static_cast<int32_t>(order.size());
+                order.push_back(j);
+            }
+            const auto& k4 = kids[static_cast<size_t>(j)];
+            for (int k = kWalkWidth - 1; k >= 0; --k)
+                if (k4[static_cast<size_t>(k)] >= 0 && inner(k4[static_cast<size_t>(k)]))
+                    dfs.push_back(node4Of[static_cast<size_t>(k4[static_cast<size_t>(k)])]);
+        }
+    };
+    std::vector<int32_t> top;
     std::deque<int32_t> bfs{0};
-    while (!bfs.empty() && static_cast<int>(order.size()) < topCount) {
+    while (!bfs.empty() && static_cast<int>(top.size()) < topCount) {
         const int32_t j = bfs.front();
         bfs.pop_front();
-        newIdx[static_cast<size_t>(j)] = static_cast<int32_t>(order.size());
-        order.push_back(j);
+        top.push_back(j);
         for (int32_t c : kids[static_cast<size_t>(j)])
             if (c >= 0 && inner(c)) bfs.push_back(node4Of[static_cast<size_t>(c)]);
     }
-    if (topPlaced != nullptr) *topPlaced = static_cast<int>(order.size());
-    std::vector<int32_t> dfs{0};
-    while (!dfs.empty()) {
-        const int32_t j = dfs.back();
-        dfs.pop_back();
-        if (newIdx[static_cast<size_t>(j)] < 0) {
-            newIdx[static_cast<size_t>(j)] = static_cast<int32_t>(order.size());
-            order.push_back(j);
-        }
-        const auto& k4 = kids[static_cast<size_t>(j)];
-        for (int k = kWalkWidth - 1; k >= 0; --k)
-            if (k4[static_cast<size_t>(k)] >= 0 && inner(k4[static_cast<size_t>(k)]))
-                dfs.push_back(node4Of[static_cast<size_t>(k4[static_cast<size_t>(k)])]);
+    number(top);
+    const bool hotFirst = hotFirstTop && nodeVisits != nullptr && nodeVisits->size() == nodes.size() && topCount > 0;
+    if (hotFirst) {
+        const std::vector<int32_t> bfIdx = newIdx;
+        const auto visitsOf = [&](int32_t j) { return (*nodeVisits)[static_cast<size_t>(kidsBvh2[static_cast<size_t>(j)])]; };
+        const auto byBf = [&](int32_t a, int32_t b) { return bfIdx[static_cast<size_t>(a)] < bfIdx[static_cast<size_t>(b)]; };
+        std::vector<int32_t> hot(n4);
+        for (size_t j = 0; j < n4; ++j) hot[j] = static_cast<int32_t>(j);
+        const size_t k = std::min(n4, static_cast<size_t>(topCount));
+        std::partial_sort(hot.begin(), hot.begin() + static_cast<std::ptrdiff_t>(k), hot.end(), [&](int32_t a, int32_t b) {
+            const double va = visitsOf(a), vb = visitsOf(b);
+            return va != vb ? va > vb : byBf(a, b);
+        });
+        hot.resize(k);
+        std::sort(hot.begin(), hot.end(), byBf);
+        top = hot;
+        number(top);
+    }
+    if (topPlaced != nullptr) *topPlaced = static_cast<int>(top.size());
+    if (wideVisits != nullptr) {
+        wideVisits->clear();
+        if (nodeVisits != nullptr && nodeVisits->size() == nodes.size())
+            for (size_t k = 0; k < n4; ++k)
+                wideVisits->push_back((*nodeVisits)[static_cast<size_t>(kidsBvh2[static_cast<size_t>(order[k])])]);
     }
     out->resize(n4);
     if (bvh2Of != nullptr) {
@@ -1829,7 +1863,7 @@
                         r2 = 1.0F - r2;
                     }
                     const v3 q = (l.tri.A + l.tri.AB * r1) + l.tri.AC * r2;
-                    rays.push_back(Ray{P, normalize(q - P), shadowW});
+                    rays.push_back(Ray{P, normalize(q - P), shadowW, length(q - P)});
                 }
                 if (p.depth >= maxDepth) continue;
                 if (diffuse && (p.depth <= 1 || U(rng) > 0.5F)) {
@@ -1854,18 +1888,22 @@
 
 constexpr float kRayCostFloor = 0.01F;
 
-std::vector<double> sampleRayNodeCosts(const std::vector<HBVHNode>& nodes, const std::vector<SampleRay>& rays) {
+std::vector<double> sampleRayNodeCosts(const std::vector<HBVHNode>& nodes, const std::vector<SampleRay>& rays,
+                                       std::vector<double>* visits) {
     std::vector<double> cost(nodes.size(), 0.0);
+    if (visits != nullptr) visits->assign(nodes.size(), 0.0);
     if (nodes.empty() || rays.empty()) return cost;
     auto inner = [&](size_t i) { return nodes[i].numPrimitives == 0 && nodes.size() > 1; };
     constexpr float floorW = kRayCostFloor;
     const unsigned hw = std::max(1u, std::min(16u, std::thread::hardware_concurrency()));
     std::vector<std::vector<double>> part(hw, std::vector<double>(nodes.size(), 0.0));
+    std::vector<std::vector<double>> partV(hw, std::vector<double>(visits != nullptr ? nodes.size() : 0, 0.0));
     std::vector<std::thread> pool;
     for (unsigned w = 0; w < hw; ++w)
         pool.emplace_back([&, w] {
             std::vector<int32_t> st;
             std::vector<double>& c = part[w];
+            std::vector<double>& cv = partV[w];
             for (size_t k = w; k < rays.size(); k += hw) {
                 const SampleRay& r = rays[k];
                 const v3 inv{1.0F / r.d.x, 1.0F / r.d.y, 1.0F / r.d.z};
@@ -1873,8 +1911,10 @@
                 while (!st.empty()) {
                     const size_t i = static_cast<size_t>(st.back());
                     st.pop_back();
-                    if (!(halfLineEntry(nodes[i].box, r.o, inv) < std::numeric_limits<float>::infinity())) continue;
+                    const float te = halfLineEntry(nodes[i].box, r.o, inv);
+                    if (!(te < std::numeric_limits<float>::infinity())) continue;
                     c[i] += r.w;
+                    if (!cv.empty() && te < r.tMax) cv[i] += r.w;
                     if (inner(i)) {
                         st.push_back(nodes[i].indexOffset);
                         st.push_back(nodes[i].indexOffset + 1);
@@ -1896,6 +1936,8 @@
         double s = 0.0;
         for (unsigned w = 0; w < hw; ++w) s += part[w][i];
         cost[i] = s + floorW * total * area(i) / rootArea;
+        if (visits != nullptr)
+            for (unsigned w = 0; w < hw; ++w) (*visits)[i] += partV[w][i];
     }
     return cost;
 }
diff --git a/mobileraytracer_amd/csrc/mrt_scene.hpp b/mobileraytracer_amd/csrc/mrt_scene.hpp
--- a/mobileraytracer_amd/csrc/mrt_scene.hpp
+++ b/mobileraytracer_amd/csrc/mrt_scene.hpp
@@ -4,6 +4,7 @@
 
 #include <functional>
 #include <istream>
+#include <limits>
 #include <string>
 #include <array>
 #include <vector>
@@ -123,16 +124,19 @@
                  int topCount = 0, int* topPlaced = nullptr, const std::vector<uint32_t>* cones = nullptr);
 bool toQuantizedBVH4(const std::vector<HBVHNode>& nodes, size_t numPrims, GRoot* root, int topCount, int* topPlaced,
                      QGrid* grid, std::vector<QNode4>* out, std::vector<int32_t>* bvh2Of = nullptr,
-                     const std::vector<double>* nodeCost = nullptr);
+                     const std::vector<double>* nodeCost = nullptr, const std::vector<double>* nodeVisits = nullptr,
+                     std::vector<double>* wideVisits = nullptr, bool hotFirstTop = true);
 std::vector<double> frameRayNodeCosts(const std::vector<HBVHNode>& nodes, const HScene& sc, const GCamera& cam,
                                       int width, int height, int maxDepth);
 struct SampleRay {
     v3 o, d;
     float w;
+    float tMax = std::numeric_limits<float>::infinity();
 };
 std::vector<SampleRay> sampleFrameRays(const std::vector<HBVHNode>& nodes, const HScene& sc, const GCamera& cam,
                                        int maxDepth);
-std::vector<double> sampleRayNodeCosts(const std::vector<HBVHNode>& nodes, const std::vector<SampleRay>& rays);
+std::vector<double> sampleRayNodeCosts(const std::vector<HBVHNode>& nodes, const std::vector<SampleRay>& rays,
+                                       std::vector<double>* visits = nullptr);
 std::vector<HBVHNode> rotateForRays(const std::vector<HBVHNode>& in, const std::vector<SampleRay>& rays, int sweeps);
 std::vector<HBVHNode> rebuildOverLeaves(const std::vector<HBVHNode>& ref, int weight = 0);
 std::vector<HBVHNode> optimizeOverLeaves(const std::vector<HBVHNode>& tree, int rounds, bool bounded = true);
diff --git a/mobileraytracer_amd/csrc/mrt_trace_ww.hpp b/mobileraytracer_amd/csrc/mrt_trace_ww.hpp
--- a/mobileraytracer_amd/csrc/mrt_trace_ww.hpp
+++ b/mobileraytracer_amd/csrc/mrt_trace_ww.hpp
@@ -300,8 +300,9 @@
 #pragma unroll
     for (int a = 0; a < 3; ++a) {
         const float ai = fabsf(iv[a]);
+        const float extent = __int_as_float(__builtin_amdgcn_readfirstlane(__float_as_int(4.0F * 65535.0F * s.qgrid.step[a])));
         ok = ok && ai >= 0x1p-40F && ai <= 0x1p90F && ai * s.qgrid.step[a] >= 0x1p-100F &&
-             fabsf(ov[a] - s.qgrid.origin[a]) <= 4.0F * 65535.0F * s.qgrid.step[a];
+             fabsf(ov[a] - s.qgrid.origin[a]) <= extent;
     }
     return ok;
 }
@@ -422,7 +423,8 @@
 __device__ __forceinline__ void traceWhileWhileQ(const DScene& s, Queue& q, Stack& st, TravCount* cnt,
                                                  const QNode4* ldsTop, int* tailBest) {
     constexpr int kSpread = kAny ? MRT_TRI_SPREAD_ANY : MRT_TRI_SPREAD;
-    __shared__ uint8_t spreadOwners[kSpread != 0 ? 192 * 4 : 1];
+    static_assert(kSpreadOwnersPerWave >= 3 * 64, "spread table: three further triangles per lane");
+    __shared__ uint8_t spreadOwners[kSpread != 0 ? kSpreadOwnersPerWave * kWalkWaves : 1];
     constexpr int kHelper = -2;
     const bool donate = s.tailDonate != 0;
     const int top = min(kWalkTop, s.triTop);
@@ -746,7 +748,7 @@
             if (m1 != 0) {
                 const uint64_t m2 = __ballot(nprim > 2 && !hit), m3 = __ballot(nprim > 3 && !hit);
                 const int c1 = __popcll(m1), c12 = c1 + __popcll(m2), total = c12 + __popcll(m3);
-                uint8_t* const owners = spreadOwners + 192 * (threadIdx.x >> 6);
+                uint8_t* const owners = spreadOwners + kSpreadOwnersPerWave * (threadIdx.x >> 6);
                 if (nprim > 1 && !hit) owners[lanesBelowIn(m1)] = static_cast<uint8_t>(lane);
                 if (nprim > 2 && !hit) owners[c1 + lanesBelowIn(m2)] = static_cast<uint8_t>(lane);
                 if (nprim > 3 && !hit) owners[c12 + lanesBelowIn(m3)] = static_cast<uint8_t>(lane);
```

After: 5431 Mrays/s (median of 6 runs). About the same (+0.6%).
